# huangzh13/StyleGAN.pytorch

Measured on AMD Instinct MI355X. Metric: img/s full G+D train step, 1024x1024 depth-9 bf16, higher is better.
Workload: dtype bf16; 1 GPU; ffhq1024: StyleGAN 1024x1024, progressive depth index 8, logistic+R1, alpha 0.5, batch 4/GPU, global batch 4; global_batch=4, parallelism=dp1

## Files before the change

### include/sgx.h

```cpp
#ifndef SGX_H
#define SGX_H
#include <stddef.h>
#include <stdint.h>
#ifdef __cplusplus
extern "C" {
#endif

enum { SGX_F32 = 0, SGX_BF16 = 1 };
enum { SGX_ACT_NONE = 0, SGX_ACT_LRELU = 1, SGX_ACT_RELU = 2 };
enum { SGX_EINVAL = -1, SGX_EUNSUPPORTED = -2, SGX_EWORKSPACE = -3 };

int sgx_version(void);
const char* sgx_last_error(void);
int sgx_clear_error(void);
int sgx_stream_wait_stream(void* waiter, void* signaler);
int sgx_selftest_tr16(void* out256, void* stream);

int sgx_prof_start(int mode, int only_of);
int sgx_prof_count(void);
int sgx_prof_get(int i, char* name, int name_cap, float* ms, double* flops, double* bytes, char* desc, int desc_cap);

int sgx_conv3x3(const void* x, const void* w, const float* bias, void* y, int B, int H, int W, int Cin, int Cout,
                int act, const void* mask, int dtype, void* stream);
int sgx_conv4x4s2_down(const void* x, const void* w, const float* bias, void* y, int B, int H, int W, int Cin,
                       int Cout, int act, int dtype, void* stream);
int sgx_conv4x4s2_up(const void* x, const void* w, void* y, int B, int H, int W, int Cin, int Cout, int dtype,
                     void* stream);
int sgx_conv_variant(int geo, const void* x, const void* w, const float* bias, void* y, int B, int H, int W, int Cin, int Cout,
                     int act, int dtype, int variant, void* stream);
size_t sgx_conv_splitk_ws_bytes(int geo, int B, int H, int W, int Cin, int Cout, int dtype);
int sgx_conv_splitk(int geo, const void* x, const void* w, const float* bias, void* y, const void* mask, int B, int H, int W, int Cin, int Cout,
                    int act, int dtype, void* ws, size_t ws_bytes, void* stream);

int sgx_conv_config(int geo, int B, int H, int W, int Cin, int Cout, int dtype, int* cfg5);
enum { SGX_PACK_S = 0, SGX_PACK_D = 1, SGX_PACK_U = 2, SGX_PACK_UF = 3 };
int sgx_pack_weight(const float* w, void* fwd, void* adj, int O, int I, int Ipad, int mode, float scale, int dtype,
                    void* stream);
#define SGX_PACK_ROW 10
int sgx_pack_weight_blocks(int O, int Ipad);
int sgx_pack_weight_multi(const void* table, int n, int total_blocks, int dtype, void* stream);
size_t sgx_wgrad_ws_bytes(int taps, int B, int H, int W, int Ck, int Cn);
int sgx_wgrad3x3_param(const void* x, const void* dy, float* dW, float* db, void* ws, size_t ws_bytes, int B, int H, int W,
                       int Cx, int Cdy, int adjoint, float scale, int O, int I, int accumulate, int dtype, void* stream);
int sgx_wgrad4x4s2_param(const void* fine, const void* coarse, float* dW, float* db, void* ws, size_t ws_bytes, int B, int H,
                         int W, int Cfine, int Ccoarse, int mode, float scale, int O, int I, int accumulate, int dtype,
                         void* stream);

int sgx_bias_act(const void* x, const float* bias, float bscale, void* y, size_t npix, int C, int act, int dtype,
                 void* stream);
int sgx_lrelu_bwd(const void* dy, const void* y, void* dx, size_t n, float slope, float scale, const float* scale_dev, int dtype,
                  void* stream);
int sgx_lrelu_bwd_bits(const void* dy, const void* bits, void* dx, size_t n, float slope, float scale, const float* scale_dev, int dtype,
                       void* stream);
int sgx_conv4x4s2_down_fade_ok(int B, int H, int W, int Cin, int Cout, int dtype);
int sgx_conv4x4s2_down_fade(const void* x, const void* w, const float* bias, const void* resid, float alpha, float beta, const float* ab_dev,
                            void* y, void* bits, int B, int H, int W, int Cin, int Cout, int dtype, void* stream);
int sgx_conv4x4s2_down_fade_rgb(const void* x, const void* w, const float* bias, const float* pimg, const float* wr, float ws, const float* rb,
                                float bs1, float bs2, float alpha, float beta, const float* ab_dev, void* y, void* bits, int B, int H, int W,
                                int Cin, int Cout, int dtype, void* stream);
size_t sgx_fade_rgb_bwd_ws_bytes(size_t npix, int C);
int sgx_fade_rgb_bwd(const void* g, const void* bits, const float* pimg, const float* wr, float ws, float bs, float alpha, float beta,
                     const float* ab_dev, void* gy, float* dwr, float* drb, int acc, float* gpimg, void* wsbuf, size_t ws_bytes, size_t npix, int C,
                     int dtype, void* stream);
int sgx_fade_rgb_bwd_finish(const void* wsbuf, size_t ws_bytes, size_t npix, int C, float ws, float bs, float beta, const float* ab_dev,
                            float* dwr, float* drb, int acc, void* stream);
int sgx_fade_rgb_bwd2(const void* ggy, const float* ggp, const void* bits, const float* wr, float ws, float alpha, float beta, const float* ab_dev,
                      void* out, size_t npix, int C, int dtype, void* stream);
int sgx_axpby(const void* a, const void* b, void* out, float alpha, float beta, size_t n, int dtype, void* stream);
int sgx_axpby_dev(const void* a, const void* b, void* out, const float* alpha_dev, const float* beta_dev, size_t n, int dtype,
                  void* stream);
int sgx_blur3x3(const void* x, void* y, int B, int H, int W, int C, int dtype, void* stream);
int sgx_blur3x3_act(const void* x, const void* z, void* y, int B, int H, int W, int C, int mode, int dtype, void* stream);
int sgx_blur3x3_bits(const void* x, const void* bits, void* y, int B, int H, int W, int C, int mode, int dtype, void* stream);
int sgx_blur_kxk(const void* x, void* y, const float* taps_host, int K, int pad, int B, int IH, int IW, int OH, int OW, int C,
                 int dtype, void* stream);
int sgx_images_u8_to_nhwc(const void* src, void* dst, const int* flip, int B, int H, int W, int src_chw, int dtype, void* stream);
int sgx_pool2(const void* x, void* y, int B, int H, int W, int C, float scale, int dtype, void* stream);
int sgx_up2(const void* x, void* y, int B, int H, int W, int C, float scale, int dtype, void* stream);
int sgx_up2_add(const void* x, const void* a, void* y, int B, int H, int W, int C, float scale, int dtype, void* stream);
size_t sgx_colsum_ws_bytes(size_t npix, int C);
int sgx_colsum(const void* x, float* out, float scale, void* ws, size_t ws_bytes, size_t npix, int C, int dtype,
               void* stream);

int sgx_rgb_in(const float* img, const float* w, int sj, int sc, float wscale, const float* bias, void* y, size_t npix,
               int C, int dtype, void* stream);
int sgx_rgb_out(const void* x, const float* w, int sj, int sc, float wscale, const float* bias, float* img, size_t npix,
                int C, int dtype, void* stream);
int sgx_rgb_in_add(const float* img, const float* w, int sj, int sc, float wscale, const void* add, void* y, size_t npix, int C, int dtype,
                   void* stream);
size_t sgx_rgb_wgrad_ws_bytes(size_t npix, int C);
int sgx_downsample_fade_rgb(const float* x, float* out, int B, int H, int W, float alpha, float beta, const float* ab_dev, void* stream);
size_t sgx_diffaug_ws_bytes(int B, int H, int W);
int sgx_diffaug(const float* x, float* y, const float* u, int B, int H, int W, int policy_bits, int adjoint, int with_bias, void* ws,
                size_t ws_bytes, void* stream);
int sgx_rgb_out_fade(const void* x, const float* w, int sj, int sc, float wscale, const float* bias, const float* low, float alpha,
                     float beta, const float* ab_dev, float* img, int B, int H, int W, int C, int dtype, void* stream);
int sgx_rgb_wgrad(const float* img, const void* f, float* dw, int sj, int sc, float wscale, void* ws, size_t ws_bytes,
                  size_t npix, int C, int dtype, void* stream);

enum { SGX_EPI_ACT = 1, SGX_EPI_NORM = 2 };
size_t sgx_gepi_ws_bytes(int B, int HW, int C);
int sgx_gepi_fwd(const void* x, const float* bias, const float* noise, const float* nw, const float* style, void* y,
                 float* mean, float* rstd, void* ws, size_t ws_bytes, const double* pre_part, int pre_npart, int B, int HW,
                 int C, int flags, int dtype, void* stream);
int sgx_blur3x3_stats_nparts(int B, int H, int W, int C, int dtype);
int sgx_conv3x3_stats_nparts(int B, int H, int W, int Cin, int Cout, int dtype);
int sgx_conv3x3_signbits_ok(int B, int H, int W, int Cin, int Cout, int dtype);
int sgx_conv3x3_signbits(const void* x, const void* w, const float* bias, void* y, void* bits, int B, int H, int W, int Cin, int Cout,
                         int act, const void* mask, int dtype, void* stream);
int sgx_conv4x4s2_up_blur_ok(int B, int H, int W, int Cin, int Cout, int dtype);
int sgx_conv4x4s2_up_blur(const void* x, const void* w, void* y, const void* mask, int B, int H, int W, int Cin, int Cout,
                          int dtype, void* stream);
int sgx_pack_upblur(const float* w, void* wc, int O, int I, int mode, int adjoint, float scale, void* stream);
int sgx_conv_upblur_ok(int B, int H, int W, int Cin, int Cout, int dtype);
int sgx_conv_upblur(const void* x, const void* wc, void* y, const void* maskbits, int B, int H, int W, int Cin, int Cout, int dtype, void* stream);
int sgx_conv4x4s2_up_blur_bits(const void* x, const void* w, void* y, const void* bits, int B, int H, int W, int Cin, int Cout,
                               int dtype, void* stream);
int sgx_conv3x3_stats(const void* x, const void* w, void* y, const float* ebias, const float* noise, const float* nw, double* part,
                      size_t part_bytes, int B, int H, int W, int Cin, int Cout, int dtype, void* stream);

int sgx_rgbconv_ok(int B, int H, int W, int C, int dtype);
int sgx_rgbconv_pack(const float* w0, float s0, const float* wr, float sr, const float* br, float bscale, void* wf, void* wd, int C,
                     void* stream);
int sgx_rgbconv_fwd(const float* img, const void* wf, const float* b0, void* y, void* bits, int B, int H, int W, int C, int epi, int ones,
                    int dtype, void* stream);
int sgx_rgbconv_tune(int fwd_variant, int nit, int dbg);
int sgx_rgbconv_dgrad(const void* gz, const void* wd, float* gi, int B, int H, int W, int C, int dtype, void* stream);
size_t sgx_rgbconv_wgrad_ws_bytes(int B, int H, int W, int C);
int sgx_rgbconv_wgrad(const float* img, const void* gz, int ones, const float* w0, float s0, const float* wr, float sr, const float* br,
                      float bscale, float* dw0, float* db0, float* dwr, float* dbr, int acc, void* ws, size_t ws_bytes, int B, int H, int W,
                      int C, int dtype, void* stream);
int sgx_blur3x3_stats(const void* x, void* y, const float* bias, const float* noise, const float* nw, double* part,
                      size_t part_bytes, int B, int H, int W, int C, int act, int dtype, void* stream);
int sgx_gepi_bwd(const void* dy, const void* x, const float* bias, const float* noise, const float* nw,
                 const float* style, const float* mean, const float* rstd, void* dx, float* dstyle, float* dnw,
                 float* dbias, void* ws, size_t ws_bytes, int B, int HW, int C, int flags, int dtype, void* stream);

int sgx_pixelnorm_fwd(const float* x, float* y, int B, int C, void* stream);
int sgx_pixelnorm_bwd(const float* dy, const float* x, float* dx, int B, int C, void* stream);
int sgx_mbstd_fwd(const void* x, void* y, int B, int HW, int C, int Cpad, int dtype, void* stream);
int sgx_mbstd_bwd(const void* dy, const void* x, void* dx, int B, int HW, int C, int Cpad, int dtype, void* stream);
int sgx_mbstd_bwd2(const void* ggx, const void* dy, const void* x, void* ddy, void* gx, int B, int HW, int C, int Cpad,
                   int dtype, void* stream);
size_t sgx_sumsq_ws_bytes(void);
int sgx_sumsq_f32(const float* x, size_t n, void* ws, size_t ws_bytes, float* out, void* stream);
int sgx_scale_dev_f32(const float* x, const float* s, float alpha, float* out, size_t n, void* stream);
int sgx_logistic_loss(const float* fake, int n_fake, const float* real, int n_real, float scale, int generator, float* loss,
                      float* g_fake, float* g_real, void* stream);
size_t sgx_gemm_ws_bytes(int M, int N, int K);
int sgx_gemm_f32(const float* A, const float* Bm, float* C, int M, int N, int K, int ta, int tb, float alpha,
                 void* ws, size_t ws_bytes, void* stream);
int sgx_linear_fwd(const float* x, const float* w, const float* bias, float* y, int B, int N, int K, float w_mul, float b_mul,
                   int act, void* stream);
int sgx_linear_bwd_data(const float* gy, const float* y_act, const float* w, float* gx, int B, int N, int K, float w_mul,
                        void* stream);
int sgx_linear_bwd_param(const float* gy, const float* y_act, const float* x, float* dw, float* db, int B, int N, int K, float w_mul,
                         float b_mul, void* stream);
#define SGX_STYLE_ROW 8
int sgx_style_fwd(const float* lm, const void* table, float* y, int G, int B, int D, int total_tiles, void* stream);
int sgx_style_bwd_data(const float* gy, const void* table, float* glm, int G, int B, int D, int max_n, void* stream);
int sgx_style_bwd_param(const float* gy, const float* lm, const void* table, float* dw, float* db, int G, int B, int D,
                        int total_tiles, void* stream);

int sgx_gepi_stats(const void* x, const float* bias, const float* noise, const float* nw, float* mean, float* rstd, void* ws, size_t ws_bytes,
                   const double* pre_part, int pre_npart, int B, int HW, int C, int flags, int dtype, void* stream);
int sgx_rgb_out_epi(const void* y, const float* ebias, const float* noise, const float* nw, const float* style, const float* mean,
                    const float* rstd, const float* w, int sj, int sc, float wscale, const float* rbias, const float* low, float alpha, float beta,
                    const float* ab_dev, float* img, int B, int H, int W, int C, int dtype, void* stream);
size_t sgx_rgb_wgrad_epi_ws_bytes(int B, int HW, int C);
int sgx_rgb_wgrad_epi(const void* y, const float* g, const float* ebias, const float* noise, const float* nw, const float* style, const float* mean,
                      const float* rstd, float* dw, float* db, int sj, int sc, float scale, float bscale, void* ws, size_t ws_bytes, int B, int HW,
                      int C, int dtype, void* stream);

int sgx_adam_multi(float* const* params, const float* const* grads, float* const* exp_avg, float* const* exp_avg_sq,
                   const int64_t* sizes, int n, float beta1, float beta2, float eps, const float* step_sizes,
                   const float* bc2_sqrts, const float* grad_scale, void* stream);
int sgx_ema_multi(float* const* tgt, const float* const* src, const int64_t* sizes, int n, float beta, void* stream);
int sgx_gradnorm_clip_coef(const float* const* grads, const int64_t* sizes, int n, float max_norm, double* partial,
                           float* out, void* stream);

#ifdef __cplusplus
}
#endif
#endif
```

### stylegan/pytorch_amd/Blocks.py

```python
import os

import torch
import torch.nn as nn

from . import functional as F
from .CustomLayers import (BlurLayer, EqualizedConv2d, EqualizedLinear, LayerEpilogue, StddevLayer, View, act_code, apply_act)
from .native import ACT_LRELU, ACT_NONE


FUSE_EPI_STATS = int(os.environ.get("SGX_FUSE_EPI_STATS", "2"))
FUSE_EPI_STATS_MIN = int(os.environ.get("SGX_FUSE_EPI_STATS_MIN", str(1 << 27)))


FUSE_BLUR_BWD = os.environ.get("SGX_FUSE_BLUR_BWD", "1") != "0"


def _lat(d, k):
    return d[k] if isinstance(d, (tuple, list)) else d[:, k]


class InputBlock(nn.Module):

    def __init__(self, nf, dlatent_size, const_input_layer, gain, use_wscale, use_noise, use_pixel_norm,
                 use_instance_norm, use_styles, activation_layer):
# ... 19 lines not shown
            x = self.const.permute(0, 2, 3, 1).to(dtype).expand(b, -1, -1, -1).contiguous()
            bias = self.bias
        else:
            x = self.dense(_lat(dlatents_in_range, 0)).view(b, self.nf, 4, 4).permute(0, 2, 3, 1).to(dtype).contiguous()
            bias = None
        x = self.epi1.forward_nhwc(x, _lat(dlatents_in_range, 0), conv_bias=bias)
        x = self.conv.forward_nhwc(x, skip_bias=True)
        return self.epi2.forward_nhwc(x, _lat(dlatents_in_range, 1), conv_bias=self.conv.scaled_bias())

    def forward(self, dlatents_in_range):
        return F.nchw_view(self.forward_nhwc(dlatents_in_range))


class GSynthesisBlock(nn.Module):

    def __init__(self, in_channels, out_channels, blur_filter, dlatent_size, gain, use_wscale, use_noise,
                 use_pixel_norm, use_instance_norm, use_styles, activation_layer):
        super().__init__()
        blur = BlurLayer(blur_filter) if blur_filter else None
        self.conv0_up = EqualizedConv2d(in_channels, out_channels, kernel_size=3, gain=gain, use_wscale=use_wscale,
                                        intermediate=blur, upscale=True)
        self.epi1 = LayerEpilogue(out_channels, dlatent_size, use_wscale, use_noise, use_pixel_norm,
                                  use_instance_norm, use_styles, activation_layer)
        self.conv1 = EqualizedConv2d(out_channels, out_channels, kernel_size=3, gain=gain, use_wscale=use_wscale)
        self.epi2 = LayerEpilogue(out_channels, dlatent_size, use_wscale, use_noise, use_pixel_norm,
                                  use_instance_norm, use_styles, activation_layer)

    def forward_nhwc(self, x, dlatents_in_range, defer_epi2=False):
        up = self.conv0_up
        if (FUSE_EPI_STATS & 1) and self.epi1._fusable and up.intermediate is not None and up.intermediate._is_121:
            b, h, w, _ = x.shape
            nin = self.epi1.noise_inputs((b, 2 * h, 2 * w, up.weight.shape[0]), x.device)
            x, part = up.forward_nhwc(x, skip_bias=True, epi_stats=(up.scaled_bias(),) + nin)
            x = self.epi1.forward_nhwc(x, _lat(dlatents_in_range, 0), conv_bias=up.scaled_bias(), noise_in=nin, pre_stats=part)
        else:
            x = up.forward_nhwc(x, skip_bias=True)
            x = self.epi1.forward_nhwc(x, _lat(dlatents_in_range, 0), conv_bias=up.scaled_bias())
        defer_epi2 = defer_epi2 and self.epi2._fusable
        if (FUSE_EPI_STATS & 2) and self.epi2._fusable and x.numel() >= FUSE_EPI_STATS_MIN:
            nin = self.epi2.noise_inputs(x.shape, x.device)
            x, part = self.conv1.forward_nhwc(x, skip_bias=True, epi_stats=(self.conv1.scaled_bias(),) + nin)
            if defer_epi2:
                return x, (self.conv1.scaled_bias(), nin[0], nin[1], self.epi2._style(_lat(dlatents_in_range, 1)), part)
            return self.epi2.forward_nhwc(x, _lat(dlatents_in_range, 1), conv_bias=self.conv1.scaled_bias(), noise_in=nin, pre_stats=part)
        if defer_epi2:
            nin = self.epi2.noise_inputs(x.shape, x.device)
            x = self.conv1.forward_nhwc(x, skip_bias=True)
            return x, (self.conv1.scaled_bias(), nin[0], nin[1], self.epi2._style(_lat(dlatents_in_range, 1)), None)
        x = self.conv1.forward_nhwc(x, skip_bias=True)
        return self.epi2.forward_nhwc(x, _lat(dlatents_in_range, 1), conv_bias=self.conv1.scaled_bias())

    def forward(self, x, dlatents_in_range):
        return F.nchw_view(self.forward_nhwc(F.nhwc(x), dlatents_in_range))


class DiscriminatorTop(nn.Module):

    def __init__(self, mbstd_group_size, mbstd_num_features, in_channels, intermediate_channels, gain, use_wscale,
                 activation_layer, resolution=4, in_channels2=None, output_features=1, last_gain=1):
        super().__init__()
        if mbstd_group_size > 1:
            self.stddev_layer = StddevLayer(mbstd_group_size, mbstd_num_features)
        else:
            self.stddev_layer = None
        if in_channels2 is None:
            in_channels2 = in_channels
        nfeat = mbstd_num_features if mbstd_group_size > 1 else 0
        self.conv = EqualizedConv2d(in_channels + nfeat, in_channels2, kernel_size=3, gain=gain, use_wscale=use_wscale)
        self.act0 = activation_layer
        self.view = View(-1)
        self.dense0 = EqualizedLinear(in_channels2 * resolution * resolution, intermediate_channels, gain=gain,
                                      use_wscale=use_wscale)
        self.act1 = activation_layer
        self.dense1 = EqualizedLinear(intermediate_channels, output_features, gain=last_gain, use_wscale=use_wscale)
        self.resolution = resolution
        self._act = act_code(activation_layer)

    def forward_nhwc(self, x):
        fused = ACT_LRELU if self._act == ACT_LRELU else ACT_NONE
        post = ACT_NONE if fused else self._act
        if self.stddev_layer is not None:
            x = self.stddev_layer.forward_nhwc(x)
        x = apply_act(self.conv.forward_nhwc(x, act=fused), post)
        b = x.shape[0]
        flat = x.permute(0, 3, 1, 2).reshape(b, -1).float()
        y = apply_act(self.dense0(flat, act=fused), post)
        return self.dense1(y)

    def forward(self, x):
        return self.forward_nhwc(F.nhwc(x))


class DiscriminatorBlock(nn.Module):

    def __init__(self, in_channels, out_channels, gain, use_wscale, activation_layer, blur_kernel):
        super().__init__()
        self.conv0 = EqualizedConv2d(in_channels, in_channels, kernel_size=3, gain=gain, use_wscale=use_wscale)
        self.act0 = activation_layer
        self.blur = BlurLayer(kernel=blur_kernel)
        self.conv1_down = EqualizedConv2d(in_channels, out_channels, kernel_size=3, gain=gain, use_wscale=use_wscale,
                                          downscale=True)
        self.act1 = activation_layer
        self._act = act_code(activation_layer)

    def fused_from_rgb_ok(self, img_shape, from_rgb, dtype):
        c0 = self.conv0
        return (FUSE_BLUR_BWD and self.blur._is_121 and self._act == ACT_LRELU and len(img_shape) == 4 and img_shape[3] == 3
                and from_rgb.kernel_size == 1 and tuple(from_rgb.weight.shape[1:]) == (3, 1, 1) and c0.b_mul == 1 and from_rgb.b_mul == 1
                and from_rgb.weight.shape[0] == c0.weight.shape[1] == c0.weight.shape[0]
                and F.rgbconv_ok(img_shape[0], img_shape[1], img_shape[2], c0.weight.shape[0], dtype))

    def forward_from_image(self, img, from_rgb, defer_out=False, fade=None):
        c0 = self.conv0
        xb, zbits = F.rgbconv_blur(img, c0.weight, c0.scaled_bias(), from_rgb.weight, from_rgb.scaled_bias(), c0.w_mul, from_rgb.w_mul)
        if fade is not None and F.conv_down_fade_ok(xb, self.conv1_down.weight.shape[0]):
            return self.conv1_down.forward_nhwc(xb, act=ACT_LRELU, x_pre=None, x_pre_bits=zbits, fade=fade), True
        y = self.conv1_down.forward_nhwc(xb, act=ACT_LRELU, defer_act=defer_out and self._act == ACT_LRELU, x_pre=None, x_pre_bits=zbits)
        return (y, False) if fade is not None else y

    def forward_nhwc(self, x, x_masked=False, defer_out=False, fade=None):
        x_masked = x_masked and self._act == ACT_LRELU
        defer_out = defer_out and self._act == ACT_LRELU
        if self.blur._is_121 and self._act == ACT_LRELU and FUSE_BLUR_BWD:
            z, zbits = self.conv0.forward_nhwc(x, act=ACT_NONE, x_masked=x_masked, sign_bits=True)
            x = F.act_blur_pass(z)
            if fade is not None and F.conv_down_fade_ok(x, self.conv1_down.weight.shape[0]):
                return self.conv1_down.forward_nhwc(x, act=ACT_LRELU, x_pre=z, x_pre_bits=zbits, fade=fade), True
            y = self.conv1_down.forward_nhwc(x, act=ACT_LRELU, defer_act=defer_out, x_pre=z, x_pre_bits=zbits)
            return (y, False) if fade is not None else y
        z = self.conv0.forward_nhwc(x, act=ACT_NONE, x_masked=x_masked)
        if self.blur._is_121 and self._act == ACT_LRELU:
            x = F.call(F.ActBlurFn, z)
        else:
            x = self.blur.forward_nhwc(apply_act(z, self._act))
        if self._act == ACT_LRELU:
            y = self.conv1_down.forward_nhwc(x, act=ACT_LRELU, defer_act=defer_out)
        else:
            y = apply_act(self.conv1_down.forward_nhwc(x, act=ACT_NONE), self._act)
        return (y, False) if fade is not None else y

    def forward(self, x):
        return F.nchw_view(self.forward_nhwc(F.nhwc(x)))
```

### stylegan/pytorch_amd/CustomLayers.py

```python
import math

import numpy as np
import torch
import torch.nn as nn

from . import functional as F
from .native import ACT_LRELU, ACT_NONE, ACT_RELU, EPI_ACT, EPI_NORM

MBSTD_CPAD = 32


def act_code(activation_layer):
    if isinstance(activation_layer, nn.LeakyReLU) and abs(activation_layer.negative_slope - 0.2) < 1e-12:
        return ACT_LRELU
    if activation_layer is torch.relu or isinstance(activation_layer, nn.ReLU):
        return ACT_RELU
    raise NotImplementedError(f"activation {activation_layer!r}: the reference offers 'lrelu' (0.2) and 'relu'")


def apply_act(x, act):
    return F.call(F.BiasActFn, x, None, 1.0, act) if act else x


class PixelNormLayer(nn.Module):
# ... 40 lines not shown
        k = torch.tensor(kernel, dtype=torch.float32)
        k = k[:, None] * k[None, :]
        k = k[None, None]
        if normalize:
            k = k / k.sum()
        if flip:
            k = k.flip(2, 3)
        self.register_buffer('kernel', k)
        self.stride = stride
        self._is_121 = (list(kernel) == [1, 2, 1]) and normalize and stride == 1
        self._is_box2 = (len(kernel) == 2 and stride == 2 and abs(float(k.sum()) - 1.0) < 1e-6
                         and float((k - k.mean()).abs().max()) < 1e-7)
        self._taps = None

    def _host_taps(self):
        ver = self.kernel._version
        if self._taps is None or self._taps[0] != ver:
            k = self.kernel.detach().float().cpu()
            self._taps = (ver, int(k.shape[2]), tuple(float(v) for v in k.reshape(-1)))
        return self._taps[1], self._taps[2]

    def forward_nhwc(self, x):
        if self._is_121:
            return F.call(F.BlurFn, x)
        if self._is_box2:
            return F.call(F.Pool2Fn, x, 0.25)
        if self.stride != 1:
            raise NotImplementedError("BlurLayer: stride 2 is built for the 2x2 box of Downscale2d only")
        K, taps = self._host_taps()
        if K > 7:
            raise NotImplementedError("BlurLayer: filters longer than 7 taps are not built")
        pad = int((K - 1) / 2)
        return F.call(F.BlurGenFn, x, taps, K, pad, x.shape[1] + 2 * pad - K + 1, x.shape[2] + 2 * pad - K + 1)

    def forward(self, x):
        return F.nchw_view(self.forward_nhwc(F.nhwc(x)))


class Downscale2d(nn.Module):

    def __init__(self, factor=2, gain=1):
        super().__init__()
        assert isinstance(factor, int) and factor >= 1
        self.factor = factor
        self.gain = gain
        if factor == 2:
            f = [np.sqrt(gain) / factor] * factor
            self.blur = BlurLayer(kernel=f, normalize=False, stride=factor)
        else:
            self.blur = None

    def forward_nhwc(self, x):
        assert self.factor == 2, "the kernel implements the factor-2 case the networks use"
        return F.call(F.Pool2Fn, x, 0.25 * float(self.gain))

    def forward(self, x):
        assert x.dim() == 4
        return F.nchw_view(self.forward_nhwc(F.nhwc(x)))


class EqualizedLinear(nn.Module):

    first_order_only = False

    def __init__(self, input_size, output_size, gain=2 ** 0.5, use_wscale=False, lrmul=1, bias=True):
        super().__init__()
        he_std = gain * input_size ** (-0.5)
        if use_wscale:
            init_std = 1.0 / lrmul
            self.w_mul = he_std * lrmul
        else:
            init_std = he_std / lrmul
            self.w_mul = lrmul
        self.weight = nn.Parameter(torch.randn(output_size, input_size) * init_std)
        if bias:
            self.bias = nn.Parameter(torch.zeros(output_size))
            self.b_mul = lrmul
        else:
            self.bias = None
            self.b_mul = 1

    def forward(self, x, act=ACT_NONE, weight=None):
        w = self.weight if weight is None else weight
        if self.first_order_only and x.dim() == 2:
            return F.linear_fused(x.float(), w, self.bias, self.w_mul, self.b_mul, act)
        return F.linear(x.float(), w, self.bias, self.w_mul, self.b_mul, act)


class EqualizedConv2d(nn.Module):

    def __init__(self, input_channels, output_channels, kernel_size, stride=1, gain=2 ** 0.5, use_wscale=False,
                 lrmul=1, bias=True, intermediate=None, upscale=False, downscale=False):
        super().__init__()
        self.upscale = Upscale2d() if upscale else None
        self.downscale = Downscale2d() if downscale else None
        he_std = gain * (input_channels * kernel_size ** 2) ** (-0.5)
        self.kernel_size = kernel_size
        if use_wscale:
            init_std = 1.0 / lrmul
            self.w_mul = he_std * lrmul
        else:
            init_std = he_std / lrmul
            self.w_mul = lrmul
        self.weight = nn.Parameter(torch.randn(output_channels, input_channels, kernel_size, kernel_size) * init_std)
        if bias:
            self.bias = nn.Parameter(torch.zeros(output_channels))
            self.b_mul = lrmul
        else:
            self.bias = None
            self.b_mul = 1
        self.intermediate = intermediate
        assert stride == 1

    def scaled_bias(self):
        if self.bias is None:
            return None
        return self.bias * self.b_mul if self.b_mul != 1 else self.bias

    def forward_nhwc(self, x, act=ACT_NONE, skip_bias=False, out_dtype=None, defer_act=False, x_masked=False, out_scale=1.0,
                     epi_stats=None, x_pre=None, sign_bits=False, x_pre_bits=None, fade=None):
        bias = None if skip_bias else self.scaled_bias()
        cin, cout = self.weight.shape[1], self.weight.shape[0]
        if self.kernel_size == 1:
            assert self.upscale is None and self.downscale is None and self.intermediate is None
            if cin == 3 and x.shape[3] == 3:
                if out_scale != 1.0:
                    y = F.call(F.RgbInFn, x.float(), self.weight, None if bias is None else bias * float(out_scale),
                               self.w_mul * float(out_scale), out_dtype or torch.float32)
                else:
                    y = F.call(F.RgbInFn, x.float(), self.weight, bias, self.w_mul, out_dtype or torch.float32)
            elif cin % 3 == 0 and cin > 3 and x.shape[3] == cin and cout != 3:
                y = None
                for k in range(0, cin, 3):
                    part = F.call(F.RgbInFn, x[..., k:k + 3].float().contiguous(), self.weight[:, k:k + 3].contiguous(),
                                  bias if k == 0 else None, self.w_mul, out_dtype or torch.float32)
                    y = part if y is None else F.call(F.AxpbyFn, y, part, 1.0, 1.0)
            elif cout == 3:
                y = F.call(F.RgbOutFn, x, self.weight, bias, self.w_mul)
            else:
                raise NotImplementedError("1x1 EqualizedConv2d is built for the to_rgb / from_rgb layers (3 channels on one side)")
            return F.call(F.BiasActFn, y, None, 1.0, act) if act else y
        assert self.kernel_size == 3
        if epi_stats is not None:
            assert skip_bias and act == ACT_NONE and self.downscale is None
            ebias, noise, nw = epi_stats
            if self.upscale is not None:
                fused = min(x.shape[1], x.shape[2]) * 2 >= 128
                y = F.conv(x, self.weight, None, "U" if fused else "UF", self.w_mul)
                assert self.intermediate is not None and self.intermediate._is_121
                return F.call(F.BlurStatsFn, y, ebias, noise, nw)
            assert self.intermediate is None
            if F.conv_stats_nparts(x, self.weight.shape[0]) > 0:
                return F.conv(x, self.weight, None, "S", self.w_mul, ipad=x.shape[3], stats=(ebias, noise, nw))
            return F.conv(x, self.weight, None, "S", self.w_mul, ipad=x.shape[3]), None
        if self.upscale is not None:
            fused = min(x.shape[1], x.shape[2]) * 2 >= 128
            mode = "U" if fused else "UF"
            if (self.intermediate is not None and self.intermediate._is_121
                    and F.conv_blur_ok(x, self.weight.shape[0], mode, False)):
                y = F.call(F.ConvBlurFn, x, self.weight, mode, float(self.w_mul), int(self.weight.shape[1]), False, None)
            else:
                y = F.conv(x, self.weight, None, mode, self.w_mul)
                if self.intermediate is not None:
                    y = self.intermediate.forward_nhwc(y)
            if bias is not None or act:
                y = F.call(F.BiasActFn, y, bias, 1.0, act)
# ... 172 lines not shown
```

### stylegan/pytorch_amd/GAN.py

```python
import contextlib
import copy
import datetime
import os
import random
import time
import timeit
from collections import OrderedDict

import numpy as np
import torch
import torch.nn as nn

from . import Losses
from . import functional as F
from .Blocks import DiscriminatorBlock, DiscriminatorTop, GSynthesisBlock, InputBlock
from .CustomLayers import EqualizedConv2d, EqualizedLinear, PixelNormLayer, Truncation, act_code, apply_act
from .data import get_data_loader
from . import native
from .native import ACT_LRELU
from .optim import FusedAdam, clip_and_step, ema_update


class DeferredLoss:

# ... 5 lines not shown
            with torch.cuda.stream(stream) if stream is not None else contextlib.nullcontext():
                t = dev_scalar.detach().reshape(1).float()
                view, slot = native.RING.take(4)
                self._host = view.view(torch.float32)
                self._host.copy_(t, non_blocking=True)
                self._event = native.RING.mark(slot, owner=self)
        else:
            self._host, self._event = dev_scalar.detach().reshape(1).float().clone(), None

    def item(self):
        if self._value is None:
            if self._event is not None:
                self._event.synchronize()
            self._value = float(self._host[0]) * self._scale
        return self._value

    __float__ = item

    def __format__(self, spec): return format(self.item(), spec)
    def __repr__(self): return repr(self.item())
    def __add__(self, o): return self.item() + float(o)
    __radd__ = __add__
    def __sub__(self, o): return self.item() - float(o)
    def __rsub__(self, o): return float(o) - self.item()
    def __mul__(self, o): return self.item() * float(o)
    __rmul__ = __mul__
    def __truediv__(self, o): return self.item() / float(o)
    def __lt__(self, o): return self.item() < float(o)
    def __gt__(self, o): return self.item() > float(o)
    def __eq__(self, o): return self.item() == float(o)
    def __abs__(self): return abs(self.item())
    def __neg__(self): return -self.item()
    def __hash__(self): return hash(self.item())


FUSE_RGB_FADE = os.environ.get("SGX_FUSE_RGB_FADE", "1") != "0"


def _nonlinearity(name):
    return {'relu': (nn.ReLU(), np.sqrt(2)), 'lrelu': (nn.LeakyReLU(negative_slope=0.2), np.sqrt(2))}[name]


def _conv_weights(module):
    ws = module.__dict__.get("_sgx_conv_weights")
    if ws is None:
        ws = [m.weight for m in module.modules() if isinstance(m, EqualizedConv2d)]
        module.__dict__["_sgx_conv_weights"] = ws
    return ws


def update_average(model_tgt, model_src, beta):
    ema_update(model_tgt, model_src, beta)


class GMapping(nn.Module):

    def __init__(self, latent_size=512, dlatent_size=512, dlatent_broadcast=None, mapping_layers=8, mapping_fmaps=512,
                 mapping_lrmul=0.01, mapping_nonlinearity='lrelu', use_wscale=True, normalize_latents=True, **kwargs):
        super().__init__()
        self.latent_size = latent_size
        self.mapping_fmaps = mapping_fmaps
        self.dlatent_size = dlatent_size
        self.dlatent_broadcast = dlatent_broadcast
        act, gain = _nonlinearity(mapping_nonlinearity)
        self._act = act_code(act)
        layers = []
        if normalize_latents:
            layers.append(('pixel_norm', PixelNormLayer()))
        layers.append(('dense0', EqualizedLinear(self.latent_size, self.mapping_fmaps, gain=gain, lrmul=mapping_lrmul,
                                                 use_wscale=use_wscale)))
        layers.append(('dense0_act', act))
        for layer_idx in range(1, mapping_layers):
            fmaps_in = self.mapping_fmaps
            fmaps_out = self.dlatent_size if layer_idx == mapping_layers - 1 else self.mapping_fmaps
            layers.append(('dense{:d}'.format(layer_idx),
                           EqualizedLinear(fmaps_in, fmaps_out, gain=gain, lrmul=mapping_lrmul, use_wscale=use_wscale)))
            layers.append(('dense{:d}_act'.format(layer_idx), act))
        self.map = nn.Sequential(OrderedDict(layers))
        self.mapping_layers = mapping_layers
        for m in self.map.modules():
            if isinstance(m, EqualizedLinear):
                m.first_order_only = True

    def forward(self, x):
        x = x.float()
        if hasattr(self.map, 'pixel_norm'):
            x = self.map.pixel_norm(x)
        for i in range(self.mapping_layers):
            dense = getattr(self.map, 'dense{:d}'.format(i))
            if self._act == ACT_LRELU:
                x = dense(x, act=ACT_LRELU)
            else:
                x = apply_act(dense(x), self._act)
        if self.dlatent_broadcast is not None:
            x = x.unsqueeze(1).expand(-1, self.dlatent_broadcast, -1)
        return x


class GSynthesis(nn.Module):

    def __init__(self, dlatent_size=512, num_channels=3, resolution=1024, fmap_base=8192, fmap_decay=1.0, fmap_max=512,
                 use_styles=True, const_input_layer=True, use_noise=True, nonlinearity='lrelu', use_wscale=True,
                 use_pixel_norm=False, use_instance_norm=True, blur_filter=None, structure='linear', act_dtype=torch.float32,
                 **kwargs):
        super().__init__()

        def nf(stage):
            return min(int(fmap_base / (2.0 ** (stage * fmap_decay))), fmap_max)

        self.structure = structure
        resolution_log2 = int(np.log2(resolution))
        assert resolution == 2 ** resolution_log2 and resolution >= 4
        self.depth = resolution_log2 - 1
        self.num_layers = resolution_log2 * 2 - 2
        self.num_styles = self.num_layers if use_styles else 1
        self.act_dtype = act_dtype
        act, gain = _nonlinearity(nonlinearity)

        self.init_block = InputBlock(nf(1), dlatent_size, const_input_layer, gain, use_wscale, use_noise, use_pixel_norm,
                                     use_instance_norm, use_styles, act)
        rgb_converters = [EqualizedConv2d(nf(1), num_channels, 1, gain=1, use_wscale=use_wscale)]
        blocks = []
        for res in range(3, resolution_log2 + 1):
            last_channels = nf(res - 2)
            channels = nf(res - 1)
            blocks.append(GSynthesisBlock(last_channels, channels, blur_filter, dlatent_size, gain, use_wscale, use_noise,
                                          use_pixel_norm, use_instance_norm, use_styles, act))
            rgb_converters.append(EqualizedConv2d(channels, num_channels, 1, gain=1, use_wscale=use_wscale))
        self.blocks = nn.ModuleList(blocks)
        self.to_rgb = nn.ModuleList(rgb_converters)
        self.temporaryUpsampler = lambda x: F.nchw_view(F.call(F.Up2Fn, F.nhwc(x), 1.0))

    def forward(self, dlatents_in, depth=0, alpha=0., labels_in=None):
        assert depth < self.depth, "Requested output depth cannot be produced"
        F.prepack(_conv_weights(self))
        dl = self._styles(dlatents_in.float(), depth)
        dt = self.act_dtype
        nblocks = len(self.blocks) if self.structure == 'fixed' else depth
        prev_arena = F.NOISE_ARENA
        if any(m.noise is None for m in self._noise_layers()):
            b = dlatents_in.shape[0]
            F.NOISE_ARENA = F.NoiseArena(b * sum(2 * (4 << k) ** 2 for k in range(nblocks + 1)), dlatents_in.device)
        try:
            return self._forward(dl, dt, depth, alpha)
        finally:
            F.NOISE_ARENA = prev_arena

    def _styles(self, dlatents, depth):
        nblocks = len(self.blocks) if self.structure == 'fixed' else depth
        epis = [self.init_block.epi1, self.init_block.epi2]
        for blk in self.blocks[:nblocks]:
            epis += [blk.epi1, blk.epi2]
        B = dlatents.shape[0]
        ok = (getattr(self.init_block, "const_input_layer", False) and B <= 32 and dlatents.shape[2] % 64 == 0
              and all(getattr(e, "_fusable", False) and e.style_mod is not None for e in epis))
        if not ok:
            return F.call(F.SplitLayersFn, dlatents)
        lins = [e.style_mod.lin for e in epis]
        meta = tuple((i, float(l.w_mul), float(l.b_mul)) for i, l in enumerate(lins))
        lm = dlatents.transpose(0, 1).contiguous()
        styles = F.call(F.GroupedStyleFn, lm, meta, *[l.weight for l in lins], *[l.bias for l in lins])
        return [F.PreStyle(s) for s in styles] + [None] * (dlatents.shape[1] - len(styles))

    def _noise_layers(self):
        ls = self.__dict__.get("_sgx_noise_layers")
        if ls is None:
            from .CustomLayers import NoiseLayer
            ls = self.__dict__["_sgx_noise_layers"] = [m for m in self.modules() if isinstance(m, NoiseLayer)]
        return ls

    def _forward(self, dl, dt, depth, alpha):
        if self.structure == 'fixed':
            x = self.init_block.forward_nhwc(dl[0:2], dt)
            rgb, last = self.to_rgb[-1], (self.blocks[-1] if len(self.blocks) else None)
            fuse_last = (F.FUSE_EPI_RGB and last is not None and last.epi2._fusable and rgb.weight.shape[0] == 3
                         and F.epi_rgb_out_ok(rgb.weight.shape[1], self.act_dtype))
            for i, block in enumerate(self.blocks):
                if fuse_last and block is last:
                    y2, (ebias, noise, nw, style, part) = block.forward_nhwc(x, dl[2 * (i + 1):2 * (i + 2)], defer_epi2=True)
                    return F.nchw_view(F.call(F.EpiRgbOutFn, y2, ebias, noise, nw, style, rgb.weight, rgb.scaled_bias(), float(rgb.w_mul), None, 1.0, part))
                x = block.forward_nhwc(x, dl[2 * (i + 1):2 * (i + 2)])
            images = rgb.forward_nhwc(x)
        elif self.structure == 'linear':
            x = self.init_block.forward_nhwc(dl[0:2], dt)
            if depth > 0:
                for i, block in enumerate(self.blocks[:depth - 1]):
                    x = block.forward_nhwc(x, dl[2 * (i + 1):2 * (i + 2)])
                prev = self.to_rgb[depth - 1]
                if F.RGB_FORK and prev.weight.shape[0] == 3 and prev.weight.shape[1] == x.shape[3]:
                    x, low = F.call(F.RgbOutForkFn, x, prev.weight, prev.scaled_bias(), prev.w_mul)
                else:
                    low = prev.forward_nhwc(x)
                rgb = self.to_rgb[depth]
                last = self.blocks[depth - 1]
                if (F.FUSE_EPI_RGB and FUSE_RGB_FADE and last.epi2._fusable and rgb.weight.shape[0] == 3 and low.dtype == torch.float32
                        and F.epi_rgb_out_ok(rgb.weight.shape[1], x.dtype)):
                    y2, (ebias, noise, nw, style, part) = last.forward_nhwc(x, dl[2 * depth:2 * (depth + 1)], defer_epi2=True)
                    return F.nchw_view(F.call(F.EpiRgbOutFn, y2, ebias, noise, nw, style, rgb.weight, rgb.scaled_bias(), float(rgb.w_mul), low,
                                              alpha if isinstance(alpha, torch.Tensor) else float(alpha), part))
                xs = last.forward_nhwc(x, dl[2 * depth:2 * (depth + 1)])
                if FUSE_RGB_FADE and rgb.weight.shape[0] == 3 and low.dtype == torch.float32:
                    images = F.call(F.RgbOutFadeFn, xs, rgb.weight, rgb.scaled_bias(), float(rgb.w_mul), low, alpha)
                else:
                    images = F.fade(rgb.forward_nhwc(xs), F.call(F.Up2Fn, low, 1.0), alpha)
            else:
                images = self.to_rgb[0].forward_nhwc(x)
        else:
            raise KeyError("Unknown structure: ", self.structure)
        return F.nchw_view(images)


class Generator(nn.Module):

    def __init__(self, resolution, latent_size=512, dlatent_size=512, conditional=False, n_classes=0, truncation_psi=0.7,
                 truncation_cutoff=8, dlatent_avg_beta=0.995, style_mixing_prob=0.9, **kwargs):
        super().__init__()
        if conditional:
            assert n_classes > 0, "Conditional generation requires n_class > 0"
            self.class_embedding = nn.Embedding(n_classes, latent_size)
            latent_size *= 2
        self.conditional = conditional
        self.style_mixing_prob = style_mixing_prob
        self.num_layers = (int(np.log2(resolution)) - 1) * 2
        self.g_mapping = GMapping(latent_size, dlatent_size, dlatent_broadcast=self.num_layers, **kwargs)
        self.g_synthesis = GSynthesis(resolution=resolution, **kwargs)
        if truncation_psi > 0:
            self.truncation = Truncation(avg_latent=torch.zeros(dlatent_size), max_layer=truncation_cutoff,
                                         threshold=truncation_psi, beta=dlatent_avg_beta)
        else:
            self.truncation = None

    _mixing_override = None
    _avg_latent_hook = None

    def draw_mixing_host(self, shape, depth):
        latents2 = torch.randn(shape)
        cur_layers = 2 * (depth + 1)
        cutoff = random.randint(1, cur_layers) if random.random() < self.style_mixing_prob else cur_layers
        return latents2, cutoff

    def draw_mixing(self, shape, depth, device):
        latents2, cutoff = self.draw_mixing_host(shape, depth)
        if device.type == "cuda":
            latents2 = native.upload(latents2.contiguous(), device)[0]
        return latents2, cutoff

    def forward(self, latents_in, depth, alpha, labels_in=None):
        if self.conditional:
            assert labels_in is not None, "Conditional discriminatin requires labels"
            latents_in = torch.cat([latents_in, self.class_embedding(labels_in)], 1)
        mixing = self.training and self.style_mixing_prob is not None and self.style_mixing_prob > 0
        if mixing:
            latents2, mixing_cutoff = self._mixing_override or self.draw_mixing(latents_in.shape, depth, latents_in.device)
            both = self.g_mapping(torch.cat([latents_in, latents2.to(latents_in.dtype)], 0))
            dlatents_in, dlatents2 = both[:latents_in.shape[0]], both[latents_in.shape[0]:]
        else:
            dlatents_in = self.g_mapping(latents_in)
        if self.training:
            if self.truncation is not None:
                self.truncation.update(dlatents_in[0, 0].detach())
                if self._avg_latent_hook is not None:
                    self._avg_latent_hook(self.truncation.avg_latent)
            if mixing:
                layer_idx = torch.arange(self.num_layers, device=latents_in.device).view(1, -1, 1)
                dlatents_in = torch.where(layer_idx < mixing_cutoff, dlatents_in, dlatents2)
            if self.truncation is not None:
                dlatents_in = self.truncation(dlatents_in)
        return self.g_synthesis(dlatents_in, depth, alpha)


class Discriminator(nn.Module):

    def __init__(self, resolution, num_channels=3, conditional=False, n_classes=0, fmap_base=8192, fmap_decay=1.0,
                 fmap_max=512, nonlinearity='lrelu', use_wscale=True, mbstd_group_size=4, mbstd_num_features=1,
                 blur_filter=None, structure='linear', act_dtype=torch.float32, diffaug_policy="", **kwargs):
        super().__init__()
        self.diffaug_policy = diffaug_policy or ""
        self._diffaug_bits = F.diffaug_policy_bits(self.diffaug_policy)
        if conditional:
            assert n_classes > 0, "Conditional Discriminator requires n_class > 0"
            num_channels *= 2
        embeddings = []

        def nf(stage):
            return min(int(fmap_base / (2.0 ** (stage * fmap_decay))), fmap_max)

        self.conditional = conditional
        self.mbstd_num_features = mbstd_num_features
        self.mbstd_group_size = mbstd_group_size
        self.structure = structure
        self.act_dtype = act_dtype
        resolution_log2 = int(np.log2(resolution))
        assert resolution == 2 ** resolution_log2 and resolution >= 4
        self.depth = resolution_log2 - 1
        act, gain = _nonlinearity(nonlinearity)

        blocks, from_rgb = [], []
        for res in range(resolution_log2, 2, -1):
            blocks.append(DiscriminatorBlock(nf(res - 1), nf(res - 2), gain=gain, use_wscale=use_wscale,
                                             activation_layer=act, blur_kernel=blur_filter))
            from_rgb.append(EqualizedConv2d(num_channels, nf(res - 1), kernel_size=1, gain=gain, use_wscale=use_wscale))
            if conditional:
                r = 2 ** res
                embeddings.append(nn.Embedding(n_classes, (num_channels // 2) * r * r))
        if conditional:
            embeddings.append(nn.Embedding(n_classes, (num_channels // 2) * 4 * 4))
            self.embeddings = nn.ModuleList(embeddings)
        self.blocks = nn.ModuleList(blocks)
        self.final_block = DiscriminatorTop(self.mbstd_group_size, self.mbstd_num_features, in_channels=nf(2),
                                            intermediate_channels=nf(2), gain=gain, use_wscale=use_wscale,
                                            activation_layer=act)
        from_rgb.append(EqualizedConv2d(num_channels, nf(2), kernel_size=1, gain=gain, use_wscale=use_wscale))
        self.from_rgb = nn.ModuleList(from_rgb)
        self.temporaryDownsampler = lambda x: F.nchw_view(F.call(F.Pool2Fn, F.nhwc(x), 0.25))

    diffaug_override = None

    def _diffaug(self, img):
        u = self.diffaug_override
        if u is None:
            u = torch.rand(img.shape[0], 7, device=img.device)
        return F.call(F.DiffAugFn, img, u, self._diffaug_bits)

    def prepack(self, depth=None, img_shape=None):
        F.prepack(_conv_weights(self))
        if depth is not None and img_shape is not None and self.structure == 'linear' and depth > 0 and not self.conditional:
            top, top_rgb = self.blocks[self.depth - depth - 1], self.from_rgb[self.depth - depth - 1]
            if top.fused_from_rgb_ok(img_shape, top_rgb, self.act_dtype):
                F.rgb_packs(top.conv0.weight, top.conv0.w_mul, top_rgb.weight, top_rgb.w_mul, top_rgb.scaled_bias())

    def forward(self, images_in, depth, alpha=1., labels_in=None):
        assert depth < self.depth, "Requested output depth cannot be produced"
        img = F.nhwc(images_in, torch.float32)
        if self._diffaug_bits and self.training:
            img = self._diffaug(img)
        self.prepack(depth, img.shape)
# ... 742 lines not shown
```

### stylegan/pytorch_amd/csrc/pointwise.hip

```cpp
#include "common.h"

static inline unsigned grid_for(size_t nvec, int block = 256) {
    size_t g = (nvec + block - 1) / block;
    static const size_t cap = [] { const char* e = getenv("SGX_GRID_CAP"); const long v = e ? atol(e) : 8192; return (size_t)(v > 0 ? v : 0x7fffffffL); }();
    if (g > cap) g = cap;
    if (g < 1) g = 1;
    return (unsigned)g;
}
static inline unsigned grid_all(size_t nvec, int block = 256) {
    size_t g = (nvec + block - 1) / block;
    static const size_t cap = [] { const char* e = getenv("SGX_GRID_ALL_CAP"); const long v = e ? atol(e) : 0; return (size_t)(v > 0 ? v : 0x7fffffffL); }();
    if (g > cap) g = cap;
    if (g < 1) g = 1;
    return (unsigned)g;
}

template <typename T>
__global__ void bias_act_kernel(const T* __restrict__ x, const float* __restrict__ bias, float bscale, T* __restrict__ y,
                                size_t nvec, int C, int act) {
    constexpr int VE = VecTraits<T>::VE;
    const int cv = C / VE;
    for (size_t i = (size_t)blockIdx.x * blockDim.x + threadIdx.x; i < nvec; i += (size_t)gridDim.x * blockDim.x) {
        float v[VE];
        VecTraits<T>::load(x + i * VE, v);
// ... 947 lines not shown
            const int e = q * 4 + j;
            v[j] = ae[j] + scale * src[((e / 3) >> 1) * 3 + e % 3];
        }
        *reinterpret_cast<float4*>(y + row * OW * 3 + q * 4) = make_float4(v[0], v[1], v[2], v[3]);
    }
}
template <typename T>
__global__ void up2_add_kernel(const T* __restrict__ x, const T* __restrict__ a, T* __restrict__ y, int B, int H, int W, int C, float scale) {
    const int OH = 2 * H, OW = 2 * W;
    const size_t n = (size_t)B * OH * OW * C;
    for (size_t i = (size_t)blockIdx.x * blockDim.x + threadIdx.x; i < n; i += (size_t)gridDim.x * blockDim.x) {
        const int c = (int)(i % C);
        size_t p = i / C;
        const int ow = (int)(p % OW); p /= OW;
        const int oh = (int)(p % OH);
        const int b = (int)(p / OH);
        y[i] = from_f<T>(to_f(a[i]) + scale * to_f(x[(((size_t)b * H + (oh >> 1)) * W + (ow >> 1)) * C + c]));
    }
}
extern "C" int sgx_up2_add(const void* x, const void* a, void* y, int B, int H, int W, int C, float scale, int dtype, void* stream) {
    hipStream_t st = (hipStream_t)stream;
    SGX_REQUIRE(x && a && y && B > 0 && H > 0 && W > 0 && C > 0, SGX_EINVAL, "up2_add: bad arguments");
    SGX_REQUIRE(dtype == SGX_F32 || dtype == SGX_BF16, SGX_EINVAL, "up2_add: bad dtype");
    const double es = dtype == SGX_F32 ? 4.0 : 2.0;
    SGX_NOTE(0.0, 9.0 * es * B * H * W * C, "up2+add B%d %dx%d C%d", B, H, W, C);
    const size_t nout = (size_t)B * H * W * 4 * C;
    if (dtype == SGX_F32 && C == 3 && (2 * W * 3) % 4 == 0)
        hipLaunchKernelGGL(up2_add_rgb_kernel, dim3(grid_all(nout / 4)), dim3(256), 0, st, (const float*)x, (const float*)a, (float*)y, B, H, W, scale);
    else if (dtype == SGX_F32)
        hipLaunchKernelGGL(up2_add_kernel<float>, dim3(grid_for(nout)), dim3(256), 0, st, (const float*)x, (const float*)a, (float*)y, B, H, W, C, scale);
    else
        hipLaunchKernelGGL(up2_add_kernel<bf16_t>, dim3(grid_for(nout)), dim3(256), 0, st, (const bf16_t*)x, (const bf16_t*)a, (bf16_t*)y, B, H, W, C, scale);
    SGX_LAUNCH_CHECK("up2_add");
    return 0;
}
extern "C" int sgx_up2(const void* x, void* y, int B, int H, int W, int C, float scale, int dtype, void* stream) {
    hipStream_t st = (hipStream_t)stream;
    SGX_NOTE(0.0, 5.0 * (dtype == SGX_F32 ? 4.0 : 2.0) * B * H * W * C, "up2 B%d %dx%d C%d", B, H, W, C);
    const size_t nout = (size_t)B * H * W * 4 * C;
    if (dtype == SGX_F32) {
        if (C % 4 == 0) hipLaunchKernelGGL((up2_kernel<float, true>), dim3(grid_all(nout / 4)), dim3(256), 0, st, (const float*)x, (float*)y, B, H, W, C, scale);
        else if (C == 3 && W % 4 == 0 && (reinterpret_cast<uintptr_t>(x) & 15) == 0 && (reinterpret_cast<uintptr_t>(y) & 15) == 0)
            hipLaunchKernelGGL(up2_rgb4_kernel, dim3(grid_all((size_t)B * H * (W / 4))), dim3(256), 0, st, (const float*)x, (float*)y, B, H, W, scale);
        else if (C == 3 && (2 * W * 3) % 4 == 0) hipLaunchKernelGGL(up2_rgb_kernel, dim3(grid_all(nout / 4)), dim3(256), 0, st, (const float*)x, (float*)y, B, H, W, scale);
        else hipLaunchKernelGGL((up2_kernel<float, false>), dim3(grid_for(nout)), dim3(256), 0, st, (const float*)x, (float*)y, B, H, W, C, scale);
    } else {
        if (C % 8 == 0) hipLaunchKernelGGL((up2_kernel<bf16_t, true>), dim3(grid_all(nout / 8)), dim3(256), 0, st, (const bf16_t*)x, (bf16_t*)y, B, H, W, C, scale);
        else hipLaunchKernelGGL((up2_kernel<bf16_t, false>), dim3(grid_for(nout)), dim3(256), 0, st, (const bf16_t*)x, (bf16_t*)y, B, H, W, C, scale);
    }
    SGX_LAUNCH_CHECK("up2");
    return 0;
}

#define COLSUM_BLOCKS 1024
template <typename T>
__global__ void colsum_stage1(const T* __restrict__ x, double* __restrict__ ws, size_t npix, int C) {
    extern __shared__ double sh[];
    const int tpr = C < 256 ? C : 256;
    const int rows = 256 / tpr;
    const int tc = threadIdx.x % tpr, tr = threadIdx.x / tpr;
    const size_t per = (npix + gridDim.x - 1) / gridDim.x;
    const size_t p0 = (size_t)blockIdx.x * per, p1 = (p0 + per < npix) ? p0 + per : npix;
    for (int cb = 0; cb < C; cb += tpr) {
        const int c = cb + tc;
        double acc = 0.0;
        if (tr < rows && c < C) {
            float part = 0.f; int cnt = 0;
            for (size_t p = p0 + tr; p < p1; p += rows) {
                part += to_f(x[p * C + c]);
                if (++cnt == 64) { acc += (double)part; part = 0.f; cnt = 0; }
            }
            acc += (double)part;
        }
        sh[threadIdx.x] = acc;
        __syncthreads();
        if (tr == 0 && c < C) {
            double s = 0.0;
            for (int r = 0; r < rows; ++r) s += sh[r * tpr + tc];
            ws[(size_t)blockIdx.x * C + c] = s;
        }
        __syncthreads();
    }
}
__global__ __launch_bounds__(256) void colsum_stage2(const double* __restrict__ ws, float* __restrict__ out, int nblk, int C, float scale) {
    __shared__ double sh[64][5];
    const int cl = threadIdx.x & 3, pl = threadIdx.x >> 2;
    const int c = blockIdx.x * 4 + cl;
    double s = 0.0;
    if (c < C)
        for (int b = pl; b < nblk; b += 64) s += ws[(size_t)b * C + c];
    sh[pl][cl] = s;
    __syncthreads();
    if (pl == 0 && c < C) {
        double t = 0.0;
        for (int k = 0; k < 64; ++k) t += sh[k][cl];
        out[c] = (float)(t * (double)scale);
    }
}
template <typename T, int NJ>
__global__ __launch_bounds__(256) void colsum_vec_stage1(const T* __restrict__ x, const float* __restrict__ img, double* __restrict__ ws,
                                                         size_t npix, int C) {
    constexpr int VE = VecTraits<T>::VE;
    extern __shared__ float shf[];
    const int cv = C / VE, rows = 256 / cv;
    const int tc = threadIdx.x % cv, tr = threadIdx.x / cv;
    const size_t per = (npix + gridDim.x - 1) / gridDim.x;
    const size_t p0 = (size_t)blockIdx.x * per, p1 = (p0 + per < npix) ? p0 + per : npix;
    float part[NJ * VE];
#pragma unroll
    for (int k = 0; k < NJ * VE; ++k) part[k] = 0.f;
    auto accum = [&](const float (&v)[VE], size_t p) {
        if (NJ == 1) {
#pragma unroll
            for (int k = 0; k < VE; ++k) part[k] += v[k];
        } else {
            const float r = img[p * 3], g = img[p * 3 + 1], b = img[p * 3 + 2];
#pragma unroll
            for (int k = 0; k < VE; ++k) { part[k] += v[k] * r; part[VE + k] += v[k] * g; part[2 * VE + k] += v[k] * b; }
        }
    };
    size_t p = p0 + tr;
    for (; p + 3 * (size_t)rows < p1; p += 4 * (size_t)rows) {
        float v0[VE], v1[VE], v2[VE], v3[VE];
        VecTraits<T>::load(x + (p * cv + tc) * VE, v0);
        VecTraits<T>::load(x + ((p + rows) * cv + tc) * VE, v1);
        VecTraits<T>::load(x + ((p + 2 * (size_t)rows) * cv + tc) * VE, v2);
        VecTraits<T>::load(x + ((p + 3 * (size_t)rows) * cv + tc) * VE, v3);
        accum(v0, p); accum(v1, p + rows); accum(v2, p + 2 * (size_t)rows); accum(v3, p + 3 * (size_t)rows);
    }
    for (; p < p1; p += rows) {
        float v[VE];
        VecTraits<T>::load(x + (p * cv + tc) * VE, v);
        accum(v, p);
    }
#pragma unroll
    for (int k = 0; k < NJ * VE; ++k) shf[threadIdx.x * NJ * VE + k] = part[k];
    __syncthreads();
    for (int o = threadIdx.x; o < cv * NJ * VE; o += 256) {
        const int c = o / (NJ * VE), k = o % (NJ * VE);
        double s = 0.0;
        for (int r = 0; r < rows; ++r) s += (double)shf[(r * cv + c) * NJ * VE + k];
        ws[((size_t)blockIdx.x * NJ + k / VE) * C + c * VE + (k % VE)] = s;
    }
}
static bool colsum_vec_ok(int C, int ve) { const int cv = C / ve; return C % ve == 0 && cv >= 1 && cv <= 256 && (cv & (cv - 1)) == 0; }

extern "C" size_t sgx_colsum_ws_bytes(size_t npix, int C) { (void)npix; return (size_t)COLSUM_BLOCKS * C * sizeof(double); }
extern "C" int sgx_colsum(const void* x, float* out, float scale, void* ws, size_t ws_bytes, size_t npix, int C, int dtype, void* stream) {
    hipStream_t st = (hipStream_t)stream;
    SGX_REQUIRE(ws_bytes >= sgx_colsum_ws_bytes(npix, C), SGX_EWORKSPACE, "colsum: workspace");
    SGX_REQUIRE(C >= 1, SGX_EINVAL, "colsum: C=%d", C);
    SGX_NOTE(0.0, (dtype == SGX_F32 ? 4.0 : 2.0) * npix * C, "colsum %zux%d", npix, C);
    int nblk = (int)((npix + 63) / 64);
    if (nblk > COLSUM_BLOCKS) nblk = COLSUM_BLOCKS;
    if (nblk < 1) nblk = 1;
    if (dtype == SGX_F32 && colsum_vec_ok(C, 4))
        hipLaunchKernelGGL((colsum_vec_stage1<float, 1>), dim3(nblk), dim3(256), 256 * 4 * sizeof(float), st, (const float*)x, (const float*)nullptr, (double*)ws, npix, C);
    else if (dtype == SGX_BF16 && colsum_vec_ok(C, 8))
        hipLaunchKernelGGL((colsum_vec_stage1<bf16_t, 1>), dim3(nblk), dim3(256), 256 * 8 * sizeof(float), st, (const bf16_t*)x, (const float*)nullptr, (double*)ws, npix, C);
    else if (dtype == SGX_F32) hipLaunchKernelGGL(colsum_stage1<float>, dim3(nblk), dim3(256), 256 * sizeof(double), st, (const float*)x, (double*)ws, npix, C);
    else hipLaunchKernelGGL(colsum_stage1<bf16_t>, dim3(nblk), dim3(256), 256 * sizeof(double), st, (const bf16_t*)x, (double*)ws, npix, C);
    SGX_LAUNCH_CHECK("colsum_stage1");
    hipLaunchKernelGGL(colsum_stage2, dim3((C + 3) / 4), dim3(256), 0, st, (const double*)ws, out, nblk, C, scale);
    SGX_LAUNCH_CHECK("colsum_stage2");
    return 0;
}

template <typename T>
__global__ void rgb_in_kernel(const float* __restrict__ img, const float* __restrict__ w, int sj, int sc, float wscale,
                              const float* __restrict__ bias, T* __restrict__ y, size_t npix, int C, const T* __restrict__ add) {
    constexpr int VE = VecTraits<T>::VE;
    const int cv = C / VE;
    const size_t nvec = npix * cv;
    const size_t i0 = (size_t)blockIdx.x * blockDim.x + threadIdx.x;
    const int c0 = (int)(i0 % cv) * VE;
    float wr[VE], wg[VE], wb[VE], bb[VE];
#pragma unroll
    for (int j = 0; j < VE; ++j) {
        wr[j] = wscale * w[(c0 + j) * sc]; wg[j] = wscale * w[sj + (c0 + j) * sc]; wb[j] = wscale * w[2 * sj + (c0 + j) * sc];
        bb[j] = bias ? bias[c0 + j] : 0.f;
    }
    for (size_t i = i0; i < nvec; i += (size_t)gridDim.x * blockDim.x) {
        const size_t p = i / cv;
        const float r = img[p * 3], g = img[p * 3 + 1], b = img[p * 3 + 2];
        float v[VE];
#pragma unroll
        for (int j = 0; j < VE; ++j) v[j] = bb[j] + (r * wr[j] + g * wg[j] + b * wb[j]);
        if (add) {
            float av[VE];
            VecTraits<T>::load(add + i * VE, av);
#pragma unroll
            for (int j = 0; j < VE; ++j) v[j] += av[j];
        }
        VecTraits<T>::store(y + i * VE, v);
    }
}
template <typename T>
__global__ __launch_bounds__(256) void rgb_in1_kernel(const float* __restrict__ img, const float* __restrict__ w, int sj, int sc, float wscale,
                                                      const float* __restrict__ bias, T* __restrict__ y, unsigned nvec, int C, const T* __restrict__ add) {
    constexpr int VE = VecTraits<T>::VE, U = 4;
    extern __shared__ float tw[];
    for (int c = threadIdx.x; c < C; c += 256) {
        tw[c] = wscale * w[c * sc]; tw[C + c] = wscale * w[sj + c * sc]; tw[2 * C + c] = wscale * w[2 * sj + c * sc];
        tw[3 * C + c] = bias ? bias[c] : 0.f;
    }
    const unsigned i0 = blockIdx.x * (256u * U) + threadIdx.x, cv = (unsigned)(C / VE);
    float r[U], g[U], b[U];
    uint4 araw[U];
#pragma unroll
    for (int u = 0; u < U; ++u) {
        const unsigned i = i0 + u * 256u;
        r[u] = g[u] = b[u] = 0.f; araw[u] = make_uint4(0u, 0u, 0u, 0u);
        if (i < nvec) {
            const size_t p = i / cv;
            r[u] = img[p * 3]; g[u] = img[p * 3 + 1]; b[u] = img[p * 3 + 2];
            if (add) araw[u] = *reinterpret_cast<const uint4*>(add + (size_t)i * VE);
        }
    }
    __syncthreads();
#pragma unroll
    for (int u = 0; u < U; ++u) {
        const unsigned i = i0 + u * 256u;
        if (i >= nvec) continue;
        const int c0 = (int)(i % cv) * VE;
        float v[VE];
#pragma unroll
        for (int j = 0; j < VE; ++j) v[j] = tw[3 * C + c0 + j] + (r[u] * tw[c0 + j] + g[u] * tw[C + c0 + j] + b[u] * tw[2 * C + c0 + j]);
        if (add) {
            const unsigned w4[4] = {araw[u].x, araw[u].y, araw[u].z, araw[u].w};
            if constexpr (sizeof(T) == 2) {
#pragma unroll
                for (int k = 0; k < 4; ++k) { v[(2 * k) % VE] += __uint_as_float(w4[k] << 16); v[(2 * k + 1) % VE] += __uint_as_float(w4[k] & 0xffff0000u); }
            } else {
#pragma unroll
                for (int k = 0; k < 4; ++k) v[k % VE] += __uint_as_float(w4[k]);
            }
        }
        VecTraits<T>::store(y + (size_t)i * VE, v);
    }
}
template <typename T>
static bool rgb_in1_launch(const float* img, const float* w, int sj, int sc, float wscale, const float* bias, T* y, size_t npix, int C, const T* add, hipStream_t st) {
    static const int on = [] { const char* e = getenv("SGX_RGB_IN1"); return e ? atoi(e) : 1; }();
    const size_t nvec = npix * (C / VecTraits<T>::VE);
    if (!on || nvec < 65536 || nvec >= 0x7fffffffull || C > 2048) return false;
    hipLaunchKernelGGL(rgb_in1_kernel<T>, dim3((unsigned)((nvec + 1023) / 1024)), dim3(256), (size_t)4 * C * sizeof(float), st, img, w, sj, sc, wscale, bias, y,
// ... 461 lines not shown
```

### stylegan/pytorch_amd/csrc/small.hip

```cpp
#include "common.h"

__global__ void pixelnorm_fwd_kernel(const float* __restrict__ x, float* __restrict__ y, int B, int C) {
    const int row = blockIdx.x * (blockDim.x / 64) + threadIdx.x / 64, lane = threadIdx.x & 63;
    if (row >= B) return;
    float ss = 0.f;
    for (int c = lane; c < C; c += 64) { const float v = x[(size_t)row * C + c]; ss += v * v; }
    ss = wave_sum(ss);
    const float r = rsqrtf(ss / C + 1e-8f);
    for (int c = lane; c < C; c += 64) y[(size_t)row * C + c] = x[(size_t)row * C + c] * r;
}
__global__ void pixelnorm_bwd_kernel(const float* __restrict__ dy, const float* __restrict__ x, float* __restrict__ dx, int B, int C) {
    const int row = blockIdx.x * (blockDim.x / 64) + threadIdx.x / 64, lane = threadIdx.x & 63;
    if (row >= B) return;
    float ss = 0.f, dot = 0.f;
    for (int c = lane; c < C; c += 64) {
        const float v = x[(size_t)row * C + c];
        ss += v * v; dot += v * dy[(size_t)row * C + c];
    }
    ss = wave_sum(ss); dot = wave_sum(dot);
    const float r = rsqrtf(ss / C + 1e-8f);
    const float k = r * r * r * dot / C;
    for (int c = lane; c < C; c += 64) dx[(size_t)row * C + c] = dy[(size_t)row * C + c] * r - x[(size_t)row * C + c] * k;
}
extern "C" int sgx_pixelnorm_fwd(const float* x, float* y, int B, int C, void* stream) {
// ... 111 lines not shown
    for (int i0 = threadIdx.x; i0 < n; i0 += MBSTD_U * blockDim.x) {
        float v[MBSTD_U][4], gg[MBSTD_U][4];
#pragma unroll
        for (int u = 0; u < MBSTD_U; ++u) {
            const int i = i0 + u * blockDim.x, ii = i < n ? i : n - 1;
#pragma unroll
            for (int g = 0; g < 4; ++g) {
                const size_t o = (size_t)((g < G ? g : 0) * M + m) * n + ii;
                v[u][g] = to_f(x[o]); gg[u][g] = to_f(ggx[o]);
            }
        }
#pragma unroll
        for (int u = 0; u < MBSTD_U; ++u)
            if (i0 + u * (int)blockDim.x < n) {
                float mu = 0.f;
                MBSTD_FOR_G(g) mu += v[u][g];
                mu /= G;
                float var = 0.f, dot = 0.f;
                MBSTD_FOR_G(g) {
                    const float d = v[u][g] - mu;
                    var += d * d;
                    dot += d * gg[u][g];
                }
                a_dd += (double)(dot / sqrtf(var / G + 1e-8f));
            }
    }
    const float k = (float)(block_sum_d(a_gy, sh) / n) / G;
    const float dstat = (float)(block_sum_d(a_dd, sh) / n) / G;
    for (int i = blockIdx.y * blockDim.x + threadIdx.x; i < n; i += gridDim.y * blockDim.x) {
        float v[4], gg[4], mu = 0.f;
#pragma unroll
        for (int g = 0; g < 4; ++g) {
            const size_t o = (size_t)((g < G ? g : 0) * M + m) * n + i;
            v[g] = to_f(x[o]); gg[g] = to_f(ggx[o]);
        }
        MBSTD_FOR_G(g) mu += v[g];
        mu /= G;
        float var = 0.f, dot = 0.f;
        MBSTD_FOR_G(g) { const float d = v[g] - mu; var += d * d; dot += d * gg[g]; }
        const float s = sqrtf(var / G + 1e-8f);
        float u[4], um = 0.f;
        MBSTD_FOR_G(g) { u[g] = gg[g] / s - dot * (v[g] - mu) / (G * s * s * s); um += u[g]; }
        um /= G;
        MBSTD_FOR_G(g) gx[(size_t)(g * M + m) * n + i] = from_f<T>(k * (u[g] - um));
    }
    mbstd_padded_copy(ggx, ddy, dstat, G, M, m, HW, C, Cpad);
}

#ifndef MBSTD_NB
#define MBSTD_NB 8
#endif
static int mbstd_check(int B, int C, int Cpad) {
    SGX_REQUIRE(B > 0 && (B < 4 || B % 4 == 0), SGX_EINVAL, "mbstd: batch %d not divisible by group size", B);
    SGX_REQUIRE(Cpad > C, SGX_EINVAL, "mbstd: Cpad must exceed C");
    return 0;
}
extern "C" int sgx_mbstd_fwd(const void* x, void* y, int B, int HW, int C, int Cpad, int dtype, void* stream) {
    int rc = mbstd_check(B, C, Cpad); if (rc) return rc;
    const int M = B / (B < 4 ? B : 4);
    if (dtype == SGX_F32) hipLaunchKernelGGL(mbstd_fwd_kernel<float>, dim3(M, MBSTD_NB), dim3(1024), 0, (hipStream_t)stream, (const float*)x, (float*)y, B, HW, C, Cpad);
    else hipLaunchKernelGGL(mbstd_fwd_kernel<bf16_t>, dim3(M, MBSTD_NB), dim3(1024), 0, (hipStream_t)stream, (const bf16_t*)x, (bf16_t*)y, B, HW, C, Cpad);
    SGX_LAUNCH_CHECK("mbstd_fwd");
    return 0;
}
extern "C" int sgx_mbstd_bwd(const void* dy, const void* x, void* dx, int B, int HW, int C, int Cpad, int dtype, void* stream) {
    int rc = mbstd_check(B, C, Cpad); if (rc) return rc;
    const int M = B / (B < 4 ? B : 4);
    if (dtype == SGX_F32) hipLaunchKernelGGL(mbstd_bwd_kernel<float>, dim3(M, MBSTD_NB), dim3(1024), 0, (hipStream_t)stream, (const float*)dy, (const float*)x, (float*)dx, B, HW, C, Cpad);
    else hipLaunchKernelGGL(mbstd_bwd_kernel<bf16_t>, dim3(M, MBSTD_NB), dim3(1024), 0, (hipStream_t)stream, (const bf16_t*)dy, (const bf16_t*)x, (bf16_t*)dx, B, HW, C, Cpad);
    SGX_LAUNCH_CHECK("mbstd_bwd");
    return 0;
}
extern "C" int sgx_mbstd_bwd2(const void* ggx, const void* dy, const void* x, void* ddy, void* gx, int B, int HW, int C, int Cpad,
                              int dtype, void* stream) {
    int rc = mbstd_check(B, C, Cpad); if (rc) return rc;
    const int M = B / (B < 4 ? B : 4);
    if (dtype == SGX_F32) hipLaunchKernelGGL(mbstd_bwd2_kernel<float>, dim3(M, MBSTD_NB), dim3(1024), 0, (hipStream_t)stream, (const float*)ggx, (const float*)dy, (const float*)x, (float*)ddy, (float*)gx, B, HW, C, Cpad);
    else hipLaunchKernelGGL(mbstd_bwd2_kernel<bf16_t>, dim3(M, MBSTD_NB), dim3(1024), 0, (hipStream_t)stream, (const bf16_t*)ggx, (const bf16_t*)dy, (const bf16_t*)x, (bf16_t*)ddy, (bf16_t*)gx, B, HW, C, Cpad);
    SGX_LAUNCH_CHECK("mbstd_bwd2");
    return 0;
}

struct GemmFuse { const float* amask; const float* bias; float bscale; int act; float* colsum; float cscale; };
template <bool VA, bool VB, bool MASK, bool TAIL>
__device__ __forceinline__ void gemm_step_load(const float* __restrict__ A, const float* __restrict__ am, const float* __restrict__ Bm,
                                               size_t arow, size_t sa_k, size_t bcol, size_t sb_k, int kk, int ke, float (&a4)[4],
                                               float (&b4)[4]) {
    if (VA && !TAIL) {
        const float4 t = *reinterpret_cast<const float4*>(A + arow + kk);
        a4[0] = t.x; a4[1] = t.y; a4[2] = t.z; a4[3] = t.w;
        if (MASK) {
            const float4 m = *reinterpret_cast<const float4*>(am + arow + kk);
            a4[0] *= lrelu_slope(m.x); a4[1] *= lrelu_slope(m.y); a4[2] *= lrelu_slope(m.z); a4[3] *= lrelu_slope(m.w);
        }
    } else {
#pragma unroll
        for (int s = 0; s < 4; ++s) {
            const int kc = (TAIL && kk + s >= ke) ? ke - 1 : kk + s;
            const size_t o = arow + kc * sa_k;
            float v = A[o];
            if (MASK) v *= lrelu_slope(am[o]);
            a4[s] = (TAIL && kk + s >= ke) ? 0.f : v;
        }
    }
    if (VB && !TAIL) {
        const float4 t = *reinterpret_cast<const float4*>(Bm + bcol + kk);
        b4[0] = t.x; b4[1] = t.y; b4[2] = t.z; b4[3] = t.w;
    } else {
#pragma unroll
        for (int s = 0; s < 4; ++s) {
            const int kc = (TAIL && kk + s >= ke) ? ke - 1 : kk + s;
            const float v = Bm[kc * sb_k + bcol];
            b4[s] = (TAIL && kk + s >= ke) ? 0.f : v;
        }
    }
}
template <int U, bool VA, bool VB, bool MASK>
__device__ __forceinline__ f32x4 gemm_wave_slice(const float* __restrict__ A, const float* __restrict__ am, const float* __restrict__ Bm,
                                                 size_t arow, size_t sa_k, size_t bcol, size_t sb_k, int kb, int ke, int q) {
    f32x4 acc = {0.f, 0.f, 0.f, 0.f};
    int k = kb;
    for (; k + 16 * U <= ke; k += 16 * U) {
        float a[U][4], b[U][4];
#pragma unroll
        for (int u = 0; u < U; ++u) gemm_step_load<VA, VB, MASK, false>(A, am, Bm, arow, sa_k, bcol, sb_k, k + 16 * u + 4 * q, ke, a[u], b[u]);
#pragma unroll
        for (int u = 0; u < U; ++u)
#pragma unroll
            for (int s = 0; s < 4; ++s) acc = __builtin_amdgcn_mfma_f32_16x16x4f32(a[u][s], b[u][s], acc, 0, 0, 0);
    }
    for (; k + 16 <= ke; k += 16) {
        float a[4], b[4];
        gemm_step_load<VA, VB, MASK, false>(A, am, Bm, arow, sa_k, bcol, sb_k, k + 4 * q, ke, a, b);
#pragma unroll
        for (int s = 0; s < 4; ++s) acc = __builtin_amdgcn_mfma_f32_16x16x4f32(a[s], b[s], acc, 0, 0, 0);
    }
    if (k < ke) {
        float a[4], b[4];
        gemm_step_load<VA, VB, MASK, true>(A, am, Bm, arow, sa_k, bcol, sb_k, k + 4 * q, ke, a, b);
#pragma unroll
        for (int s = 0; s < 4; ++s) acc = __builtin_amdgcn_mfma_f32_16x16x4f32(a[s], b[s], acc, 0, 0, 0);
    }
    return acc;
}
template <int U>
__global__ __launch_bounds__(256) void gemm_f32_kernel(const float* __restrict__ A, const float* __restrict__ Bm, float* __restrict__ Cm,
                                                       int M, int N, int K, int ta, int tb, float alpha, GemmFuse fu) {
    __shared__ float red[4][16][17];
    const int lane = threadIdx.x & 63, wave = threadIdx.x >> 6, q = lane >> 4, l15 = lane & 15;
    const int i0 = blockIdx.y * 16, j0 = blockIdx.x * 16;
    const int ic = i0 + l15 < M ? i0 + l15 : M - 1, jc = j0 + l15 < N ? j0 + l15 : N - 1;
    const int kz = ((K + (int)gridDim.z - 1) / (int)gridDim.z + 15) / 16 * 16;
    const int kz0 = blockIdx.z * kz, kz1 = (kz0 + kz < K) ? kz0 + kz : K;
    const int kper = (((kz1 > kz0 ? kz1 - kz0 : 0) + 3) / 4 + 15) / 16 * 16;
    const int kb = kz0 + wave * kper, ke = (kb + kper < kz1) ? kb + kper : kz1;
    Cm += (size_t)blockIdx.z * M * N;
    const size_t sa_i = ta ? 1 : (size_t)K, sa_k = ta ? (size_t)M : 1;
    const size_t sb_k = tb ? 1 : (size_t)N, sb_j = tb ? (size_t)K : 1;
    const size_t arow = ic * sa_i, bcol = jc * sb_j;
    const bool va = !ta && (K % 4 == 0), vb = tb && (K % 4 == 0);
    f32x4 acc;
#define GEMM_SLICE(VA, VB, MK) acc = gemm_wave_slice<U, VA, VB, MK>(A, fu.amask, Bm, arow, sa_k, bcol, sb_k, kb, ke, q)
    if (fu.amask) {
        if (va) { if (vb) GEMM_SLICE(true, true, true); else GEMM_SLICE(true, false, true); }
        else    { if (vb) GEMM_SLICE(false, true, true); else GEMM_SLICE(false, false, true); }
    } else {
        if (va) { if (vb) GEMM_SLICE(true, true, false); else GEMM_SLICE(true, false, false); }
        else    { if (vb) GEMM_SLICE(false, true, false); else GEMM_SLICE(false, false, false); }
    }
#undef GEMM_SLICE
#pragma unroll
    for (int r = 0; r < 4; ++r) red[wave][q * 4 + r][l15] = acc[r];
    __syncthreads();
    const int r = threadIdx.x >> 4, c = threadIdx.x & 15;
    if (threadIdx.x < 256 && i0 + r < M && j0 + c < N) {
        const float s = ((red[0][r][c] + red[1][r][c]) + red[2][r][c]) + red[3][r][c];
        float v = alpha * s;
        if (fu.bias) v += fu.bscale * fu.bias[j0 + c];
        if (fu.act == SGX_ACT_LRELU) v = lrelu(v);
        Cm[(size_t)(i0 + r) * N + j0 + c] = v;
    }
    if (fu.colsum && blockIdx.x == 0 && blockIdx.z == 0 && threadIdx.x < 16 && i0 + (int)threadIdx.x < M) {
        const int row = i0 + threadIdx.x;
        float t = 0.f;
        int k = 0;
        for (; k + 8 <= K; k += 8) {
            float v[8], m[8];
#pragma unroll
            for (int u = 0; u < 8; ++u) {
                const size_t o = row * sa_i + (k + u) * sa_k;
                v[u] = A[o];
                m[u] = fu.amask ? fu.amask[o] : 1.f;
            }
#pragma unroll
            for (int u = 0; u < 8; ++u) t += fu.amask ? v[u] * lrelu_slope(m[u]) : v[u];
        }
        for (; k < K; ++k) {
            const size_t o = row * sa_i + k * sa_k;
            t += fu.amask ? A[o] * lrelu_slope(fu.amask[o]) : A[o];
        }
        fu.colsum[row] = fu.cscale * t;
    }
}
__global__ __launch_bounds__(256) void gemm_outer_kernel(const float* __restrict__ A, const float* __restrict__ Bm, float* __restrict__ Cm,
                                                         int M, int N, int K, size_t sa_i, size_t sa_k, float alpha) {
    const size_t idx = (size_t)blockIdx.x * 256 + threadIdx.x, n4 = (size_t)N / 4;
    if (idx >= (size_t)M * n4) return;
    const size_t i = idx / n4, j = (idx % n4) * 4;
    float a[4];
    float4 b[4];
#pragma unroll
    for (int k = 0; k < 4; ++k) {
        const int kc = k < K ? k : 0;
        a[k] = A[i * sa_i + kc * sa_k];
        b[k] = *reinterpret_cast<const float4*>(Bm + (size_t)kc * N + j);
    }
    float4 acc = {0.f, 0.f, 0.f, 0.f};
#pragma unroll
    for (int k = 0; k < 4; ++k)
        if (k < K) {
            acc.x = fmaf(a[k], b[k].x, acc.x); acc.y = fmaf(a[k], b[k].y, acc.y); acc.z = fmaf(a[k], b[k].z, acc.z); acc.w = fmaf(a[k], b[k].w, acc.w);
        }
    acc.x *= alpha; acc.y *= alpha; acc.z *= alpha; acc.w *= alpha;
    *reinterpret_cast<float4*>(Cm + i * N + j) = acc;
}
__global__ void gemm_splitk_reduce(const float* __restrict__ part, float* __restrict__ Cm, int MN, int splits, float alpha) {
    const int i = blockIdx.x * blockDim.x + threadIdx.x;
    if (i >= MN) return;
    float s = 0.f;
    for (int z = 0; z < splits; ++z) s += part[(size_t)z * MN + i];
    Cm[i] = alpha * s;
}
static int gemm_splits(int M, int N, int K) {
    const int tiles = ((M + 15) / 16) * ((N + 15) / 16);
    if (tiles >= 256 || K < 1024) return 1;
    int s = K / 256, cap = (512 + tiles - 1) / tiles;
    if (s > cap) s = cap;
    return s < 1 ? 1 : s;
}
extern "C" size_t sgx_gemm_ws_bytes(int M, int N, int K) {
    const int s = gemm_splits(M, N, K);
    return s > 1 ? (size_t)s * M * N * sizeof(float) : 0;
}
static int gemm_launch(const float* A, const float* Bm, float* C, int M, int N, int K, int ta, int tb, float alpha, GemmFuse fu, void* ws,
                       size_t ws_bytes, hipStream_t st) {
    SGX_REQUIRE(M > 0 && N > 0 && K > 0, SGX_EINVAL, "gemm: bad shape %d %d %d", M, N, K);
    int splits = gemm_splits(M, N, K);
    if (splits > 1 && (!ws || ws_bytes < (size_t)splits * M * N * sizeof(float) || fu.bias || fu.act || fu.colsum)) splits = 1;
    SGX_NOTE(2.0 * M * N * K, 4.0 * ((double)M * K + (double)K * N + (double)M * N), "gemm %dx%dx%d t%d%d%s", M, N, K, ta, tb,
             fu.amask || fu.bias || fu.colsum ? " fused" : "");
    const bool fused = fu.amask || fu.bias || fu.act || fu.colsum;
    if (K <= 4 && !tb && N % 4 == 0 && !fused && ((uintptr_t)Bm | (uintptr_t)C) % 16 == 0) {
        const size_t n = (size_t)M * (N / 4);
        hipLaunchKernelGGL(gemm_outer_kernel, dim3((unsigned)((n + 255) / 256)), dim3(256), 0, st, A, Bm, C, M, N, K, ta ? (size_t)1 : (size_t)K,
                           ta ? (size_t)M : (size_t)1, alpha);
        SGX_LAUNCH_CHECK("gemm_outer");
        return 0;
    }
    const int ksplit = (K + splits - 1) / splits;
    auto kern = ksplit >= 512 ? gemm_f32_kernel<8> : gemm_f32_kernel<1>;
    if (splits == 1) {
        hipLaunchKernelGGL(kern, dim3((N + 15) / 16, (M + 15) / 16, 1), dim3(256), 0, st, A, Bm, C, M, N, K, ta, tb, alpha, fu);
        SGX_LAUNCH_CHECK("gemm_f32");
        return 0;
    }
    hipLaunchKernelGGL(kern, dim3((N + 15) / 16, (M + 15) / 16, splits), dim3(256), 0, st, A, Bm, (float*)ws, M, N, K, ta, tb, 1.0f, fu);
    SGX_LAUNCH_CHECK("gemm_f32");
    hipLaunchKernelGGL(gemm_splitk_reduce, dim3((M * N + 255) / 256), dim3(256), 0, st, (const float*)ws, C, M * N, splits, alpha);
    SGX_LAUNCH_CHECK("gemm_splitk_reduce");
    return 0;
}
extern "C" int sgx_gemm_f32(const float* A, const float* Bm, float* C, int M, int N, int K, int ta, int tb, float alpha, void* ws,
                            size_t ws_bytes, void* stream) {
    return gemm_launch(A, Bm, C, M, N, K, ta, tb, alpha, GemmFuse{nullptr, nullptr, 0.f, SGX_ACT_NONE, nullptr, 0.f}, ws, ws_bytes,
                       (hipStream_t)stream);
}
extern "C" int sgx_linear_fwd(const float* x, const float* w, const float* bias, float* y, int B, int N, int K, float w_mul, float b_mul,
                              int act, void* stream) {
    return gemm_launch(x, w, y, B, N, K, 0, 1, w_mul, GemmFuse{nullptr, bias, b_mul, act, nullptr, 0.f}, nullptr, 0, (hipStream_t)stream);
}
extern "C" int sgx_linear_bwd_data(const float* gy, const float* y_act, const float* w, float* gx, int B, int N, int K, float w_mul,
                                   void* stream) {
    return gemm_launch(gy, w, gx, B, K, N, 0, 0, w_mul, GemmFuse{y_act, nullptr, 0.f, SGX_ACT_NONE, nullptr, 0.f}, nullptr, 0,
                       (hipStream_t)stream);
}
extern "C" int sgx_linear_bwd_param(const float* gy, const float* y_act, const float* x, float* dw, float* db, int B, int N, int K,
                                    float w_mul, float b_mul, void* stream) {
    return gemm_launch(gy, x, dw, N, K, B, 1, 0, w_mul, GemmFuse{y_act, nullptr, 0.f, SGX_ACT_NONE, db, b_mul}, nullptr, 0,
                       (hipStream_t)stream);
}

#define STYLE_MAXB 32
__device__ __forceinline__ int style_group(const long long* __restrict__ tab, int G, unsigned tile) {
    if (G <= 64) {
        const int l = threadIdx.x & 63;
        const bool le = l < G && (unsigned)tab[(l < G ? l : 0) * SGX_STYLE_ROW + 4] <= tile;
        return __builtin_amdgcn_readfirstlane(__popcll(__ballot(le)) - 1);
    }
    int g = 0;
    while (g + 1 < G && (unsigned)tab[(g + 1) * SGX_STYLE_ROW + 4] <= tile) ++g;
    return g;
}
template <int MB>
__global__ __launch_bounds__(256) void style_fwd_kernel(const float* __restrict__ lm, const long long* __restrict__ tab, float* __restrict__ y,
                                                        int G, int B, int D) {
    extern __shared__ float xs[];
    const int g = style_group(tab, G, blockIdx.x);
    const long long* r = tab + (size_t)g * SGX_STYLE_ROW;
    const float* W = reinterpret_cast<const float*>(r[0]);
    const float* bias = reinterpret_cast<const float*>(r[1]);
    const int N = (int)r[2], layer = (int)r[7];
    const float w_mul = __uint_as_float((unsigned)r[5]), b_mul = __uint_as_float((unsigned)r[6]);
    const float* x = lm + (size_t)layer * B * D;
    const int col = threadIdx.x >> 4, kl = threadIdx.x & 15;
    const int n = ((int)blockIdx.x - (int)r[4]) * 16 + col;
    constexpr int STYLE_U = 8;
    const float* wrow = W + (size_t)(n < N ? n : N - 1) * D;
    float4 w[STYLE_U];
#pragma unroll
    for (int u = 0; u < STYLE_U; ++u) { const int k = kl * 4 + 64 * u; w[u] = *reinterpret_cast<const float4*>(wrow + (k < D ? k : D - 4)); }
    for (int i = threadIdx.x; i < B * D / 4; i += 256) reinterpret_cast<float4*>(xs)[i] = reinterpret_cast<const float4*>(x)[i];
    __syncthreads();
    float acc[MB];
#pragma unroll
    for (int b = 0; b < MB; ++b) acc[b] = 0.f;
    for (int k0 = kl * 4; k0 < D; k0 += 64 * STYLE_U) {
        if (k0 != kl * 4) {
#pragma unroll
            for (int u = 0; u < STYLE_U; ++u) { const int k = k0 + 64 * u; w[u] = *reinterpret_cast<const float4*>(wrow + (k < D ? k : D - 4)); }
        }
#pragma unroll
        for (int u = 0; u < STYLE_U; ++u) {
            const int k = k0 + 64 * u;
            if (k < D) {
#pragma unroll
                for (int b = 0; b < MB; ++b)
                    if (b < B) {
                        const float4 v = *reinterpret_cast<const float4*>(xs + b * D + k);
                        acc[b] += (w[u].x * v.x + w[u].y * v.y) + (w[u].z * v.z + w[u].w * v.w);
                    }
            }
        }
    }
#pragma unroll
    for (int b = 0; b < MB; ++b)
        if (b < B) {
#pragma unroll
            for (int o = 8; o > 0; o >>= 1) acc[b] += __shfl_xor(acc[b], o, 64);
        }
    if (n < N && kl == 0) {
        const float bb = bias ? b_mul * bias[n] : 0.f;
        float* yo = y + (size_t)r[3] + n;
#pragma unroll
        for (int b = 0; b < MB; ++b)
            if (b < B) yo[(size_t)b * N] = w_mul * acc[b] + bb;
    }
}
template <int MB>
// ... 67 lines not shown
        const int b = i / 64, kl = i % 64, k = blockIdx.x * 64 + kl;
        if (k < D) {
            const float sum = (part[(0 * B + b) * 64 + kl] + part[(1 * B + b) * 64 + kl]) + (part[(2 * B + b) * 64 + kl] + part[(3 * B + b) * 64 + kl]);
            glm[((size_t)layer * B + b) * D + k] = w_mul * sum;
        }
    }
}
template <int MB>
__global__ __launch_bounds__(256) void style_bwd_param_kernel(const float* __restrict__ gy, const float* __restrict__ lm,
                                                              const long long* __restrict__ tab, float* __restrict__ dw,
                                                              float* __restrict__ db, int G, int B, int D) {
    __shared__ float gs[MB][16];
    const int g = style_group(tab, G, blockIdx.x);
    const long long* r = tab + (size_t)g * SGX_STYLE_ROW;
    const int N = (int)r[2], layer = (int)r[7];
    const float w_mul = __uint_as_float((unsigned)r[5]), b_mul = __uint_as_float((unsigned)r[6]);
    const int n0 = ((int)blockIdx.x - (int)r[4]) * 16;
    const size_t noff = (size_t)r[3] / B;
    const float* gyg = gy + (size_t)r[3];
    for (int i = threadIdx.x; i < B * 16; i += 256) {
        const int b = i / 16, j = i % 16;
        gs[b][j] = (n0 + j < N) ? gyg[(size_t)b * N + n0 + j] : 0.f;
    }
    __syncthreads();
    const float* x = lm + (size_t)layer * B * D;
    for (int k = threadIdx.x; k < D; k += 256) {
        float xv[MB];
#pragma unroll
        for (int b = 0; b < MB; ++b) xv[b] = b < B ? x[(size_t)b * D + k] : 0.f;
#pragma unroll
        for (int j = 0; j < 16; ++j)
            if (n0 + j < N) {
                float s = 0.f;
#pragma unroll
                for (int b = 0; b < MB; ++b)
                    if (b < B) s += gs[b][j] * xv[b];
                dw[(noff + n0 + j) * D + k] = w_mul * s;
            }
    }
    if (db && threadIdx.x < 16 && n0 + (int)threadIdx.x < N) {
        float s = 0.f;
        for (int b = 0; b < B; ++b) s += gs[b][threadIdx.x];
        db[noff + n0 + threadIdx.x] = b_mul * s;
    }
}
static int style_check(int G, int B, int D) {
    SGX_REQUIRE(G > 0 && B > 0 && B <= STYLE_MAXB && D > 0 && D % 64 == 0, SGX_EUNSUPPORTED, "style affines: G=%d B=%d D=%d", G, B, D);
    return 0;
}
extern "C" int sgx_style_fwd(const float* lm, const void* table, float* y, int G, int B, int D, int total_tiles, void* stream) {
    int rc = style_check(G, B, D); if (rc) return rc;
    SGX_NOTE(0.0, 0.0, "style_fwd G%d B%d", G, B);
    if (B <= 4) hipLaunchKernelGGL(style_fwd_kernel<4>, dim3(total_tiles), dim3(256), (size_t)B * D * sizeof(float), (hipStream_t)stream, lm, (const long long*)table, y, G, B, D);
    else if (B <= 8) hipLaunchKernelGGL(style_fwd_kernel<8>, dim3(total_tiles), dim3(256), (size_t)B * D * sizeof(float), (hipStream_t)stream, lm, (const long long*)table, y, G, B, D);
    else if (B <= 16) hipLaunchKernelGGL(style_fwd_kernel<16>, dim3(total_tiles), dim3(256), (size_t)B * D * sizeof(float), (hipStream_t)stream, lm, (const long long*)table, y, G, B, D);
    else hipLaunchKernelGGL(style_fwd_kernel<32>, dim3(total_tiles), dim3(256), (size_t)B * D * sizeof(float), (hipStream_t)stream, lm, (const long long*)table, y, G, B, D);
    SGX_LAUNCH_CHECK("style_fwd");
    return 0;
}
extern "C" int sgx_style_bwd_data(const float* gy, const void* table, float* glm, int G, int B, int D, int max_n, void* stream) {
    int rc = style_check(G, B, D); if (rc) return rc;
    const int mb = B <= 4 ? 4 : (B <= 8 ? 8 : (B <= 16 ? 16 : 32));
    const size_t a = (size_t)mb * max_n, b = (size_t)4 * B * 64;
    SGX_NOTE(0.0, 0.0, "style_bwd_data G%d B%d", G, B);
    if (B <= 4) hipLaunchKernelGGL(style_bwd_data_kernel<4>, dim3(D / 64, G), dim3(256), (a > b ? a : b) * sizeof(float), (hipStream_t)stream, gy, (const long long*)table, glm, G, B, D);
    else if (B <= 8) hipLaunchKernelGGL(style_bwd_data_kernel<8>, dim3(D / 64, G), dim3(256), (a > b ? a : b) * sizeof(float), (hipStream_t)stream, gy, (const long long*)table, glm, G, B, D);
    else if (B <= 16) hipLaunchKernelGGL(style_bwd_data_kernel<16>, dim3(D / 64, G), dim3(256), (a > b ? a : b) * sizeof(float), (hipStream_t)stream, gy, (const long long*)table, glm, G, B, D);
    else hipLaunchKernelGGL(style_bwd_data_kernel<32>, dim3(D / 64, G), dim3(256), (a > b ? a : b) * sizeof(float), (hipStream_t)stream, gy, (const long long*)table, glm, G, B, D);
    SGX_LAUNCH_CHECK("style_bwd_data");
    return 0;
}
extern "C" int sgx_style_bwd_param(const float* gy, const float* lm, const void* table, float* dw, float* db, int G, int B, int D,
                                   int total_tiles, void* stream) {
    int rc = style_check(G, B, D); if (rc) return rc;
    SGX_NOTE(0.0, 0.0, "style_bwd_param G%d B%d", G, B);
    if (B <= 4) hipLaunchKernelGGL(style_bwd_param_kernel<4>, dim3(total_tiles), dim3(256), 0, (hipStream_t)stream, gy, lm, (const long long*)table, dw, db, G, B, D);
    else if (B <= 8) hipLaunchKernelGGL(style_bwd_param_kernel<8>, dim3(total_tiles), dim3(256), 0, (hipStream_t)stream, gy, lm, (const long long*)table, dw, db, G, B, D);
    else if (B <= 16) hipLaunchKernelGGL(style_bwd_param_kernel<16>, dim3(total_tiles), dim3(256), 0, (hipStream_t)stream, gy, lm, (const long long*)table, dw, db, G, B, D);
    else hipLaunchKernelGGL(style_bwd_param_kernel<32>, dim3(total_tiles), dim3(256), 0, (hipStream_t)stream, gy, lm, (const long long*)table, dw, db, G, B, D);
    SGX_LAUNCH_CHECK("style_bwd_param");
    return 0;
}

#define SUMSQ_BLOCKS 1024
__global__ __launch_bounds__(256) void sumsq_f32_stage1(const float* __restrict__ x, size_t n, double* __restrict__ partial) {
    __shared__ double sh[16];
    const size_t nvec = n / 4;
    double acc = 0.0;
    float part = 0.f; int cnt = 0;
    const size_t gs = (size_t)gridDim.x * 256;
    size_t i = (size_t)blockIdx.x * 256 + threadIdx.x;
    for (; i + 3 * gs < nvec; i += 4 * gs) {
        const float4 v0 = reinterpret_cast<const float4*>(x)[i], v1 = reinterpret_cast<const float4*>(x)[i + gs];
        const float4 v2 = reinterpret_cast<const float4*>(x)[i + 2 * gs], v3 = reinterpret_cast<const float4*>(x)[i + 3 * gs];
        part += ((v0.x * v0.x + v0.y * v0.y) + (v0.z * v0.z + v0.w * v0.w)) + ((v1.x * v1.x + v1.y * v1.y) + (v1.z * v1.z + v1.w * v1.w));
        part += ((v2.x * v2.x + v2.y * v2.y) + (v2.z * v2.z + v2.w * v2.w)) + ((v3.x * v3.x + v3.y * v3.y) + (v3.z * v3.z + v3.w * v3.w));
        if (++cnt == 4) { acc += (double)part; part = 0.f; cnt = 0; }
    }
    for (; i < nvec; i += gs) {
        const float4 v = reinterpret_cast<const float4*>(x)[i];
        part += (v.x * v.x + v.y * v.y) + (v.z * v.z + v.w * v.w);
    }
    if (blockIdx.x == 0 && threadIdx.x == 0)
        for (size_t i = nvec * 4; i < n; ++i) part += x[i] * x[i];
    acc += (double)part;
    const double s = block_sum_d(acc, sh);
    if (threadIdx.x == 0) partial[blockIdx.x] = s;
}
__global__ __launch_bounds__(256) void sumsq_f32_stage2(const double* __restrict__ partial, int nblk, float* __restrict__ out) {
    __shared__ double sh[16];
    double acc = 0.0;
    for (int i = threadIdx.x; i < nblk; i += 256) acc += partial[i];
    const double s = block_sum_d(acc, sh);
    if (threadIdx.x == 0) out[0] = (float)s;
}
extern "C" size_t sgx_sumsq_ws_bytes(void) { return SUMSQ_BLOCKS * sizeof(double); }
extern "C" int sgx_sumsq_f32(const float* x, size_t n, void* ws, size_t ws_bytes, float* out, void* stream) {
    SGX_REQUIRE(ws_bytes >= SUMSQ_BLOCKS * sizeof(double), SGX_EWORKSPACE, "sumsq: workspace");
    int nblk = (int)((n / 4 + 255) / 256);
    if (nblk > SUMSQ_BLOCKS) nblk = SUMSQ_BLOCKS;
    if (nblk < 1) nblk = 1;
    hipLaunchKernelGGL(sumsq_f32_stage1, dim3(nblk), dim3(256), 0, (hipStream_t)stream, x, n, (double*)ws);
    SGX_LAUNCH_CHECK("sumsq_stage1");
    hipLaunchKernelGGL(sumsq_f32_stage2, dim3(1), dim3(256), 0, (hipStream_t)stream, (const double*)ws, nblk, out);
    SGX_LAUNCH_CHECK("sumsq_stage2");
    return 0;
}
__device__ __forceinline__ float softplus_f(float x) { return x > 20.f ? x : log1pf(expf(x)); }
__device__ __forceinline__ float sigmoid_f(float x) { return 1.f / (1.f + expf(-x)); }
__global__ void logistic_loss_kernel(const float* __restrict__ fake, int nf, const float* __restrict__ real, int nr, float scale, int gen,
                                     float* __restrict__ loss, float* __restrict__ gfake, float* __restrict__ greal) {
    const int l = threadIdx.x;
    float sf = 0.f, sr = 0.f;
    const float sgn = gen ? -1.f : 1.f;
    for (int i = l; i < nf; i += 64) {
        const float x = sgn * fake[i];
        sf += softplus_f(x);
        gfake[i] = sgn * scale * sigmoid_f(x) / (float)nf;
    }
    for (int i = l; i < nr; i += 64) {
        const float x = -real[i];
        sr += softplus_f(x);
        greal[i] = -scale * sigmoid_f(x) / (float)nr;
    }
    sf = wave_sum(sf); sr = wave_sum(sr);
    if (l == 0) loss[0] = scale * (sf / (float)(nf > 0 ? nf : 1) + (nr > 0 ? sr / (float)nr : 0.f));
}
extern "C" int sgx_logistic_loss(const float* fake, int n_fake, const float* real, int n_real, float scale, int generator, float* loss,
                                 float* g_fake, float* g_real, void* stream) {
    SGX_REQUIRE(fake && n_fake > 0 && loss && g_fake, SGX_EINVAL, "logistic_loss: fake logits, loss and g_fake are required");
    SGX_REQUIRE(generator ? n_real == 0 : (real && g_real && n_real > 0), SGX_EINVAL, "logistic_loss: real logits %s", generator ? "are not part of the generator loss" : "are required");
    hipLaunchKernelGGL(logistic_loss_kernel, dim3(1), dim3(64), 0, (hipStream_t)stream, fake, n_fake, real, n_real, scale, generator, loss, g_fake, g_real);
    SGX_LAUNCH_CHECK("logistic_loss");
    return 0;
}
__global__ void scale_dev_kernel(const float* __restrict__ x, const float* __restrict__ s, float alpha, float* __restrict__ out, size_t n) {
    const float k = alpha * s[0];
    const size_t nvec = n / 4;
    for (size_t i = (size_t)blockIdx.x * blockDim.x + threadIdx.x; i < nvec; i += (size_t)gridDim.x * blockDim.x) {
        float4 v = reinterpret_cast<const float4*>(x)[i];
        v.x *= k; v.y *= k; v.z *= k; v.w *= k;
        reinterpret_cast<float4*>(out)[i] = v;
    }
    if (blockIdx.x == 0 && threadIdx.x == 0)
        for (size_t i = nvec * 4; i < n; ++i) out[i] = k * x[i];
}
// ... 9 lines not shown
```

### stylegan/pytorch_amd/functional.py

```python
import contextlib
import functools
import os
import weakref

import numpy as np
import torch
from torch.autograd import Function
from torch.autograd.function import once_differentiable

from . import native as N

_DATA_GRAD_ONLY = 0


@contextlib.contextmanager
def data_grad_only():
    global _DATA_GRAD_ONLY
    _DATA_GRAD_ONLY += 1
    try:
        yield
    finally:
        _DATA_GRAD_ONLY -= 1


# ... 938 lines not shown
        ctx.save_for_backward(x, weight, None, None, x_pre, x_pre_bits, bits, alpha if dev else None, pimg, wr)
        return y

    @staticmethod
    def backward(ctx, g):
        g = _c(g)
        bits, alpha_dev, pimg, wr = ctx.saved_tensors[6:10]
        alpha, beta, ws, bs = ctx.fade
        br = ctx.br_ref()
        need_img = ctx.needs_input_grad[3]
        want_w = ctx.needs_input_grad[4] and not _DATA_GRAD_ONLY
        want_b = br is not None and ctx.needs_input_grad[5] and not _DATA_GRAD_ONLY
        gpimg = gwr = gbr = None
        if torch.is_grad_enabled() and FUSE_FADE_BWD2 and not want_w and not want_b:
            gy, gpimg = FadeRgbBwdFn.apply(g, bits, pimg, wr, ws, alpha, beta, alpha_dev, bool(need_img))
        elif torch.is_grad_enabled():
            if alpha_dev is not None:
                g_res = _bcall(ScaleDevFn, g, alpha_dev[1:2])
                gy = _bcall(LReluBwdBitsFn, g, bits, 0.2, alpha_dev[0:1])
            else:
                g_res = g if beta == 1.0 else _bcall(ScaleFn, g, beta)
                gy = _bcall(LReluBwdBitsFn, g, bits, 0.2, alpha)
            if need_img:
                gpimg = _bcall(RgbOutFn, g_res, wr, None, ws)
            if want_w:
                gwr = _bcall(RgbWgradFn, pimg, g_res, wr, ws)
            if want_b:
                gbr = _bcall(ColSumFn, g_res, bs)
        else:
            L = N.lib()
            C = g.shape[-1]
            npix = g.numel() // C
            accum = _ACCUM_PARAM_GRADS and wr.is_leaf and (br is None or br.is_leaf)
            acc = 0
            dw = db = None
            if want_w and accum and wr.grad is not None:
                dw, acc = wr.grad, acc | 1
            if want_b and accum and br.grad is not None:
                db, acc = br.grad, acc | 2
            gy = torch.empty_like(g)
            if need_img:
                gpimg = torch.empty_like(pimg)
            wsb = L.sgx_fade_rgb_bwd_ws_bytes(npix, C)
            wsp = N.workspace(wsb, g.device)
            dev = alpha_dev is not None
            side = _PARAM_GRAD_STREAM if (accum and (want_w or want_b)) else None
            cur_raw = N.stream()
            if side is not None and side.cuda_stream == cur_raw:
                side = None
            if side is None:
                if want_w and dw is None:
                    dw = torch.empty(wr.shape, dtype=torch.float32, device=g.device)
                if want_b and db is None:
                    db = torch.empty(br.shape, dtype=torch.float32, device=g.device)
            N.check(L.sgx_fade_rgb_bwd(N.ptr(g), N.ptr(bits), N.ptr(pimg), N.ptr(_c(wr.detach())), ws, bs, 0.0 if dev else alpha, 0.0 if dev else beta,
                                       alpha_dev.data_ptr() if dev else None, N.ptr(gy), None if side is not None else N.ptr(dw),
                                       None if side is not None else N.ptr(db), acc, N.ptr(gpimg), N.ptr(wsp), wsb, npix, C,
                                       N.dt(g), cur_raw), "sgx_fade_rgb_bwd")
            if side is not None:
                fresh = []

                def finish():
                    nonlocal dw, db
                    if want_w and dw is None:
                        dw = torch.empty(wr.shape, dtype=torch.float32, device=g.device); fresh.append(dw)
                    if want_b and db is None:
                        db = torch.empty(br.shape, dtype=torch.float32, device=g.device); fresh.append(db)
                    N.check(L.sgx_fade_rgb_bwd_finish(N.ptr(wsp), wsb, npix, C, ws, bs, 0.0 if dev else beta, alpha_dev.data_ptr() if dev else None,
                                                      N.ptr(dw), N.ptr(db), acc, N.stream()), "sgx_fade_rgb_bwd_finish")
                _fork_to(side, cur_raw, finish, reads=(wsp,) + ((alpha_dev,) if dev else ()), fresh=fresh)
            if accum:
                for p_, d_ in ((wr, dw), (br, db)):
                    if d_ is not None:
                        if p_.grad is None:
                            p_.grad = d_
                        if GRAD_NOTE is not None:
                            GRAD_NOTE(p_)
            else:
                gwr, gbr = dw, db
        out = ConvFn.backward(ctx, gy)
        return (out[0], out[1], out[2], gpimg, gwr, gbr) + (None,) * 9


class ColSumFn(Function):

    @staticmethod
    def forward(ctx, x, scale):
        x = _c(x)
        C = x.shape[-1]
        npix = x.numel() // C
        out = torch.empty((C,), dtype=torch.float32, device=x.device)
        L = N.lib()
        ws = N.workspace(L.sgx_colsum_ws_bytes(npix, C), x.device)
        N.check(L.sgx_colsum(N.ptr(x), N.ptr(out), float(scale), N.ptr(ws), ws.numel(), npix, C, N.dt(x), N.stream()), "sgx_colsum")
        ctx.shape, ctx.dtype, ctx.scale = x.shape, x.dtype, float(scale)
        return out

    @staticmethod
    def backward(ctx, g):
        return (g * ctx.scale).to(ctx.dtype).expand(ctx.shape), None


class BiasActFn(Function):

    @staticmethod
    def forward(ctx, x, bias, bscale, act):
        x = _c(x)
        C = x.shape[-1]
        y = torch.empty_like(x)
        N.check(N.lib().sgx_bias_act(N.ptr(x), N.ptr(None if bias is None else _c(bias.detach())), float(bscale), N.ptr(y),
                                     x.numel() // C, C, act, N.dt(x), N.stream()), "sgx_bias_act")
        ctx.act, ctx.has_bias, ctx.bscale = act, bias is not None, float(bscale)
        ctx.save_for_backward(y if act else None)
        return y

    @staticmethod
    def backward(ctx, g):
        (y,) = ctx.saved_tensors
        g = _c(g)
        if ctx.act:
            g = _bcall(LReluBwdFn, g, y, 0.0 if ctx.act == N.ACT_RELU else 0.2, 1.0)
        gb = None
        if ctx.has_bias and ctx.needs_input_grad[1] and not _DATA_GRAD_ONLY:
            gb = _bcall(ColSumFn, g, ctx.bscale)
        return g, gb, None, None


class ScaleFn(Function):
    @staticmethod
    def forward(ctx, x, s):
        x = _c(x)
        out = torch.empty_like(x)
        N.check(N.lib().sgx_axpby(N.ptr(x), None, N.ptr(out), float(s), 0.0, x.numel(), N.dt(x), N.stream()), "sgx_axpby")
        ctx.s = float(s)
        return out

    @staticmethod
    def backward(ctx, g):
        return _bcall(ScaleFn, g, ctx.s), None


class AxpbyFn(Function):

    @staticmethod
    def forward(ctx, a, b, alpha, beta, a_act=False):
        a, b = _c(a), _c(b)
        assert a.shape == b.shape and a.dtype == b.dtype
        out = torch.empty_like(a)
        N.check(N.lib().sgx_axpby(N.ptr(a), N.ptr(b), N.ptr(out), float(alpha), float(beta), a.numel(), N.dt(a), N.stream()), "sgx_axpby")
        ctx.alpha, ctx.beta, ctx.a_act = float(alpha), float(beta), bool(a_act)
        ctx.save_for_backward(a if a_act else None)
        return out

    @staticmethod
    def backward(ctx, g):
        (a,) = ctx.saved_tensors
        ga = gb = None
        if ctx.needs_input_grad[0]:
            ga = _bcall(LReluBwdFn, g, a, 0.2, ctx.alpha) if ctx.a_act else _bcall(ScaleFn, g, ctx.alpha)
        if ctx.needs_input_grad[1]:
            gb = g if ctx.beta == 1.0 else _bcall(ScaleFn, g, ctx.beta)
        return ga, gb, None, None, None


class ScaleDevFn(Function):

    @staticmethod
    def forward(ctx, x, s):
        x = _c(x)
        out = torch.empty_like(x)
        N.check(N.lib().sgx_axpby_dev(N.ptr(x), None, N.ptr(out), s.data_ptr(), None, x.numel(), N.dt(x), N.stream()), "sgx_axpby_dev")
        ctx.s = s
        return out

    @staticmethod
    def backward(ctx, g):
        return _bcall(ScaleDevFn, g, ctx.s), None


class FadeFn(Function):

    @staticmethod
    def forward(ctx, a, b, ab, a_act=False):
        a, b = _c(a), _c(b)
        assert a.shape == b.shape and a.dtype == b.dtype and ab.dtype == torch.float32 and ab.numel() == 2 and ab.is_contiguous()
        out = torch.empty_like(a)
        N.check(N.lib().sgx_axpby_dev(N.ptr(a), N.ptr(b), N.ptr(out), ab.data_ptr(), ab.data_ptr() + 4, a.numel(), N.dt(a), N.stream()),
                "sgx_axpby_dev")
        ctx.ab, ctx.a_act = ab, bool(a_act)
        ctx.save_for_backward(a if a_act else None)
        return out

    @staticmethod
    def backward(ctx, g):
        (a,) = ctx.saved_tensors
        ga = gb = None
        if ctx.needs_input_grad[0]:
            ga = _bcall(LReluBwdFn, g, a, 0.2, ctx.ab[0:1]) if ctx.a_act else _bcall(ScaleDevFn, g, ctx.ab[0:1])
        if ctx.needs_input_grad[1]:
            gb = _bcall(ScaleDevFn, g, ctx.ab[1:2])
        return ga, gb, None, None


def fade(a, b, alpha, a_act=False, b_prescaled=False):
    if isinstance(alpha, torch.Tensor):
        assert not b_prescaled
        return call(FadeFn, a, b, alpha, bool(a_act))
# ... 553 lines not shown
        dx = torch.empty_like(x)
        N.check(N.lib().sgx_mbstd_bwd(N.ptr(gy), N.ptr(x), N.ptr(dx), B, H * W, C, gy.shape[3], N.dt(x), N.stream()), "sgx_mbstd_bwd")
        ctx.save_for_backward(gy, x)
        return dx

    @staticmethod
    @once_differentiable
    def backward(ctx, ggx):
        gy, x = ctx.saved_tensors
        ggx = _c(ggx)
        B, H, W, C = x.shape
        ddy = torch.empty_like(gy)
        gx = torch.empty_like(x)
        N.check(N.lib().sgx_mbstd_bwd2(N.ptr(ggx), N.ptr(gy), N.ptr(x), N.ptr(ddy), N.ptr(gx), B, H * W, C, gy.shape[3], N.dt(x),
                                       N.stream()), "sgx_mbstd_bwd2")
        return ddy, gx


def _dense_view(x):
    if x.is_contiguous():
        return x, None
    if x.dim() == 4 and x.permute(0, 2, 3, 1).is_contiguous():
        return x.permute(0, 2, 3, 1), (0, 3, 1, 2)
    return x.contiguous(), None


class SumSqFn(Function):

    @staticmethod
    def forward(ctx, x):
        xv, back = _dense_view(x.detach())
        if xv.dtype != torch.float32:
            raise N.SgxError("SumSqFn expects fp32 (image gradients)")
        L = N.lib()
        out = torch.empty((), dtype=torch.float32, device=x.device)
        ws = N.workspace(L.sgx_sumsq_ws_bytes(), x.device)
        N.check(L.sgx_sumsq_f32(N.ptr(xv), xv.numel(), N.ptr(ws), ws.numel(), N.ptr(out), N.stream()), "sgx_sumsq_f32")
        ctx.back = back
        ctx.save_for_backward(xv)
        return out

    @staticmethod
    @once_differentiable
    def backward(ctx, g):
        (xv,) = ctx.saved_tensors
        gx = torch.empty_like(xv)
        N.check(N.lib().sgx_scale_dev_f32(N.ptr(xv), N.ptr(_c(g.float())), 2.0, N.ptr(gx), xv.numel(), N.stream()), "sgx_scale_dev_f32")
        return gx if ctx.back is None else gx.permute(*ctx.back)


class LogisticLossFn(Function):

    @staticmethod
    def forward(ctx, fake, real, scale, generator):
        f = _c(fake.detach().reshape(-1))
        r = None if real is None else _c(real.detach().reshape(-1))
        if f.dtype != torch.float32 or (r is not None and r.dtype != torch.float32):
            raise N.SgxError("LogisticLossFn: fp32 logits expected")
        loss = torch.empty((), dtype=torch.float32, device=f.device)
        gf = torch.empty_like(f)
        gr = None if r is None else torch.empty_like(r)
        N.check(N.lib().sgx_logistic_loss(N.ptr(f), f.numel(), N.ptr(r), 0 if r is None else r.numel(), float(scale), int(bool(generator)),
                                          N.ptr(loss), N.ptr(gf), N.ptr(gr), N.stream()), "sgx_logistic_loss")
        ctx.save_for_backward(gf, gr)
        ctx.shapes = (fake.shape, None if real is None else real.shape)
        return loss

    @staticmethod
    @once_differentiable
    def backward(ctx, g):
        gf, gr = ctx.saved_tensors
        g = _c(g.float())
        out = []
        for t, shape in zip((gf, gr), ctx.shapes):
            if t is None:
                out.append(None)
                continue
            o = torch.empty_like(t)
            N.check(N.lib().sgx_scale_dev_f32(N.ptr(t), N.ptr(g), 1.0, N.ptr(o), t.numel(), N.stream()), "sgx_scale_dev_f32")
            out.append(o.view(shape))
        return out[0], out[1], None, None


class MatMulFn(Function):

    @staticmethod
    def forward(ctx, A, Bm, ta, tb, alpha):
        A, Bm = _c(A), _c(Bm)
        assert A.dtype == torch.float32 and Bm.dtype == torch.float32
        M, K = (A.shape[1], A.shape[0]) if ta else (A.shape[0], A.shape[1])
        K2, Nn = (Bm.shape[1], Bm.shape[0]) if tb else (Bm.shape[0], Bm.shape[1])
        assert K == K2, (A.shape, Bm.shape, ta, tb)
        C = torch.empty((M, Nn), dtype=torch.float32, device=A.device)
        wsb = N.lib().sgx_gemm_ws_bytes(M, Nn, K)
        ws = N.workspace(wsb, A.device) if wsb else None
        N.check(N.lib().sgx_gemm_f32(N.ptr(A), N.ptr(Bm), N.ptr(C), M, Nn, K, int(ta), int(tb), float(alpha), N.ptr(ws), wsb, N.stream()), "sgx_gemm_f32")
        ctx.ta, ctx.tb, ctx.alpha = int(ta), int(tb), float(alpha)
        ctx.save_for_backward(A, Bm)
        return C

    @staticmethod
    def backward(ctx, gC):
        A, Bm = ctx.saved_tensors
        ta, tb, al = ctx.ta, ctx.tb, ctx.alpha
        gA = gB = None
        if ctx.needs_input_grad[0]:
            gA = _bcall(MatMulFn, gC, Bm, 0, 1 - tb, al) if not ta else _bcall(MatMulFn, Bm, gC, tb, 1, al)
        if ctx.needs_input_grad[1] and not _DATA_GRAD_ONLY:
            gB = _bcall(MatMulFn, A, gC, 1 - ta, 0, al) if not tb else _bcall(MatMulFn, gC, A, 1, ta, al)
        return gA, gB, None, None, None


class LinearFn(Function):

    @staticmethod
    def forward(ctx, x, weight, bias, w_mul, b_mul, act):
        x, weight = _c(x), _c(weight)
        assert x.dtype == torch.float32 and weight.dtype == torch.float32 and x.dim() == 2
        B, K = x.shape
        Nn = weight.shape[0]
        assert weight.shape[1] == K
        y = torch.empty((B, Nn), dtype=torch.float32, device=x.device)
        N.check(N.lib().sgx_linear_fwd(N.ptr(x), N.ptr(weight), None if bias is None else N.ptr(_c(bias.detach())), N.ptr(y), B, Nn, K,
                                       float(w_mul), float(b_mul), int(act), N.stream()), "sgx_linear_fwd")
        ctx.cfg = (float(w_mul), float(b_mul), int(act), bias is not None)
        ctx.save_for_backward(x, weight, y if act else None)
        return y

    @staticmethod
    @once_differentiable
    def backward(ctx, gy):
        x, weight, y = ctx.saved_tensors
        w_mul, b_mul, act, has_bias = ctx.cfg
        gy = _c(gy)
        B, K = x.shape
        Nn = weight.shape[0]
        L = N.lib()
        gx = gw = gb = None
        if ctx.needs_input_grad[0]:
            gx = torch.empty_like(x)
            N.check(L.sgx_linear_bwd_data(N.ptr(gy), N.ptr(y), N.ptr(weight), N.ptr(gx), B, Nn, K, w_mul, N.stream()), "sgx_linear_bwd_data")
        if ctx.needs_input_grad[1] or (has_bias and ctx.needs_input_grad[2]):
            gw = torch.empty_like(weight)
            gb = torch.empty((Nn,), dtype=torch.float32, device=x.device) if has_bias else None
            N.check(L.sgx_linear_bwd_param(N.ptr(gy), N.ptr(y), N.ptr(x), N.ptr(gw), N.ptr(gb), B, Nn, K, w_mul, b_mul, N.stream()),
                    "sgx_linear_bwd_param")
        return gx, gw, gb, None, None, None


def linear_fused(x, weight, bias, w_mul, b_mul, act=N.ACT_NONE):
    return call(LinearFn, x, weight, bias, float(w_mul), float(b_mul), int(act))


class SplitLayersFn(Function):

    @staticmethod
    def forward(ctx, dl):
        lm = dl.transpose(0, 1).contiguous()
        ctx.L = lm.shape[0]
        return tuple(lm.unbind(0))

    @staticmethod
    def backward(ctx, *grads):
        ref = next(g for g in grads if g is not None)
        return torch.stack([g if g is not None else torch.zeros_like(ref) for g in grads], dim=1)


class PreStyle:
    __slots__ = ("style",)

    def __init__(self, style):
        self.style = style


_STYLE_TABLES = {}


class GroupedStyleFn(Function):

    @staticmethod
    def forward(ctx, lm, meta, *params):
        G = len(meta)
        ws, bs = params[:G], params[G:]
        lm = _c(lm)
        L_, B, D = lm.shape
        key = (tuple(w.data_ptr() for w in ws), tuple(b.data_ptr() for b in bs), meta, B)
        ent = _STYLE_TABLES.get(key)
        if ent is None:
            rows, yoff, tile = [], 0, 0
            for (layer, w_mul, b_mul), w, b in zip(meta, ws, bs):
                n = w.shape[0]
                assert w.shape[1] == D and w.is_contiguous() and w.dtype == torch.float32
                rows.append([w.data_ptr(), b.data_ptr(), n, yoff, tile, int(np.float32(w_mul).view(np.uint32)),
                             int(np.float32(b_mul).view(np.uint32)), layer])
                yoff += B * n; tile += (n + 15) // 16
            table, _ = N.upload(torch.tensor(rows, dtype=torch.int64), lm.device)
            ent = _STYLE_TABLES[key] = (table, [r[2] for r in rows], [r[3] for r in rows], yoff, tile)
        table, ns, yoffs, ytotal, tiles = ent
        y = torch.empty(ytotal, dtype=torch.float32, device=lm.device)
        N.check(N.lib().sgx_style_fwd(N.ptr(lm), N.ptr(table), N.ptr(y), G, B, D, tiles, N.stream()), "sgx_style_fwd")
        ctx.ent, ctx.G, ctx.shape = ent, G, (L_, B, D)
        ctx.save_for_backward(lm)
        return tuple(y[o:o + B * n].view(B, n) for o, n in zip(yoffs, ns))

    @staticmethod
    @once_differentiable
    def backward(ctx, *gys):
        (lm,) = ctx.saved_tensors
        table, ns, yoffs, ytotal, tiles = ctx.ent
        L_, B, D = ctx.shape
        G = ctx.G
        gy = torch.cat([(g if g is not None else torch.zeros(B, n, device=lm.device)).reshape(-1) for g, n in zip(gys, ns)])
        L = N.lib()
        glm = None
        if ctx.needs_input_grad[0]:
            glm = torch.zeros_like(lm) if G < L_ else torch.empty_like(lm)
            N.check(L.sgx_style_bwd_data(N.ptr(gy), N.ptr(table), N.ptr(glm), G, B, D, max(ns), N.stream()), "sgx_style_bwd_data")
        ntot = sum(ns)
        dw = torch.empty((ntot, D), dtype=torch.float32, device=lm.device)
        db = torch.empty((ntot,), dtype=torch.float32, device=lm.device)
        N.check(L.sgx_style_bwd_param(N.ptr(gy), N.ptr(lm), N.ptr(table), N.ptr(dw), N.ptr(db), G, B, D, tiles, N.stream()),
                "sgx_style_bwd_param")
        offs = [o // B for o in yoffs]
        gws = tuple(dw[o:o + n] for o, n in zip(offs, ns))
        gbs = tuple(db[o:o + n] for o, n in zip(offs, ns))
        return (glm, None) + gws + gbs


class NoiseArena:

    def __init__(self, numel, device):
        self.buf = torch.randn(int(numel), device=device, dtype=torch.float32)
        self.off = 0

    def take(self, b, h, w):
        n = b * h * w
        if self.off + n > self.buf.numel():
            return torch.randn(b, 1, h, w, device=self.buf.device, dtype=torch.float32)
        out = self.buf[self.off:self.off + n].view(b, 1, h, w)
        self.off += n
        return out


NOISE_ARENA = None


def linear(x, weight, bias, w_mul, b_mul, act=N.ACT_NONE):
    y = call(MatMulFn, x, weight, 0, 1, w_mul)
# ... 118 lines not shown
```

### stylegan/pytorch_amd/native.py

```python
import ctypes
import os
import subprocess
import threading

import torch

_HERE = os.path.dirname(os.path.abspath(__file__))
LIB_PATH = os.environ.get("SGX_HIP_LIB") or os.path.join(_HERE, "libsgx_hip.so")
CSRC = os.path.join(_HERE, "csrc")

F32, BF16 = 0, 1
ACT_NONE, ACT_LRELU, ACT_RELU = 0, 1, 2
EPI_ACT, EPI_NORM = 1, 2
PACK_S, PACK_D, PACK_U, PACK_UF = 0, 1, 2, 3

_lib = None
_lock = threading.Lock()

c_void_p, c_int, c_float, c_size_t = ctypes.c_void_p, ctypes.c_int, ctypes.c_float, ctypes.c_size_t
P, I, F, Z = c_void_p, c_int, c_float, c_size_t

SIGNATURES = {
    "sgx_version": (I, []),
    "sgx_last_error": (ctypes.c_char_p, []),
    "sgx_clear_error": (I, []),
    "sgx_stream_wait_stream": (I, [P, P]),
    "sgx_conv3x3": (I, [P, P, P, P, I, I, I, I, I, I, P, I, P]),
    "sgx_conv_variant": (I, [I, P, P, P, P, I, I, I, I, I, I, I, I, P]),
    "sgx_conv4x4s2_down": (I, [P, P, P, P, I, I, I, I, I, I, I, P]),
    "sgx_conv4x4s2_up": (I, [P, P, P, I, I, I, I, I, I, P]),
    "sgx_wgrad_ws_bytes": (Z, [I, I, I, I, I, I]),
    "sgx_images_u8_to_nhwc": (I, [P, P, P, I, I, I, I, I, P]),
    "sgx_selftest_tr16": (I, [P, P]),
    "sgx_conv_splitk_ws_bytes": (Z, [I, I, I, I, I, I, I]),
    "sgx_conv_splitk": (I, [I, P, P, P, P, P, I, I, I, I, I, I, I, P, Z, P]),
    "sgx_conv_config": (I, [I, I, I, I, I, I, I, P]),
    "sgx_prof_start": (I, [I, I]),
    "sgx_prof_count": (I, []),
    "sgx_prof_get": (I, [I, P, I, P, P, P, P, I]),
    "sgx_pack_weight": (I, [P, P, P, I, I, I, I, F, I, P]),
    "sgx_pack_weight_multi": (I, [P, I, I, I, P]),
    "sgx_pack_weight_blocks": (I, [I, I]),
    "sgx_wgrad3x3_param": (I, [P, P, P, P, P, Z, I, I, I, I, I, I, F, I, I, I, I, P]),
    "sgx_wgrad4x4s2_param": (I, [P, P, P, P, P, Z, I, I, I, I, I, I, F, I, I, I, I, P]),
    "sgx_bias_act": (I, [P, P, F, P, Z, I, I, I, P]),
    "sgx_lrelu_bwd": (I, [P, P, P, Z, F, F, P, I, P]),
    "sgx_lrelu_bwd_bits": (I, [P, P, P, Z, F, F, P, I, P]),
    "sgx_conv4x4s2_down_fade_ok": (I, [I, I, I, I, I, I]),
    "sgx_conv4x4s2_down_fade": (I, [P, P, P, P, F, F, P, P, P, I, I, I, I, I, I, P]),
    "sgx_conv4x4s2_down_fade_rgb": (I, [P, P, P, P, P, F, P, F, F, F, F, P, P, P, I, I, I, I, I, I, P]),
    "sgx_fade_rgb_bwd_ws_bytes": (Z, [Z, I]),
    "sgx_fade_rgb_bwd": (I, [P, P, P, P, F, F, F, F, P, P, P, P, I, P, P, Z, Z, I, I, P]),
    "sgx_fade_rgb_bwd_finish": (I, [P, Z, Z, I, F, F, F, P, P, P, I, P]),
    "sgx_fade_rgb_bwd2": (I, [P, P, P, P, F, F, F, P, P, Z, I, I, P]),
    "sgx_axpby": (I, [P, P, P, F, F, Z, I, P]),
    "sgx_axpby_dev": (I, [P, P, P, P, P, Z, I, P]),
    "sgx_blur3x3": (I, [P, P, I, I, I, I, I, P]),
    "sgx_blur3x3_act": (I, [P, P, P, I, I, I, I, I, I, P]),
    "sgx_blur_kxk": (I, [P, P, P, I, I, I, I, I, I, I, I, I, P]),
    "sgx_pool2": (I, [P, P, I, I, I, I, F, I, P]),
    "sgx_up2": (I, [P, P, I, I, I, I, F, I, P]),
    "sgx_up2_add": (I, [P, P, P, I, I, I, I, F, I, P]),
    "sgx_colsum_ws_bytes": (Z, [Z, I]),
    "sgx_colsum": (I, [P, P, F, P, Z, Z, I, I, P]),
    "sgx_rgb_in": (I, [P, P, I, I, F, P, P, Z, I, I, P]),
    "sgx_rgb_in_add": (I, [P, P, I, I, F, P, P, Z, I, I, P]),
    "sgx_rgb_out": (I, [P, P, I, I, F, P, P, Z, I, I, P]),
    "sgx_downsample_fade_rgb": (I, [P, P, I, I, I, F, F, P, P]),
    "sgx_diffaug_ws_bytes": (Z, [I, I, I]),
    "sgx_diffaug": (I, [P, P, P, I, I, I, I, I, I, P, Z, P]),
    "sgx_rgb_out_fade": (I, [P, P, I, I, F, P, P, F, F, P, P, I, I, I, I, I, P]),
    "sgx_rgb_wgrad_ws_bytes": (Z, [Z, I]),
    "sgx_rgb_wgrad": (I, [P, P, P, I, I, F, P, Z, Z, I, I, P]),
    "sgx_gepi_ws_bytes": (Z, [I, I, I]),
    "sgx_gepi_fwd": (I, [P, P, P, P, P, P, P, P, P, Z, P, I, I, I, I, I, I, P]),
    "sgx_gepi_stats": (I, [P, P, P, P, P, P, P, Z, P, I, I, I, I, I, I, P]),
    "sgx_rgb_out_epi": (I, [P, P, P, P, P, P, P, P, I, I, F, P, P, F, F, P, P, I, I, I, I, I, P]),
    "sgx_rgb_wgrad_epi_ws_bytes": (Z, [I, I, I]),
    "sgx_rgb_wgrad_epi": (I, [P, P, P, P, P, P, P, P, P, P, I, I, F, F, P, Z, I, I, I, I, P]),
    "sgx_blur3x3_stats_nparts": (I, [I, I, I, I, I]),
    "sgx_conv3x3_stats_nparts": (I, [I, I, I, I, I, I]),
    "sgx_conv3x3_signbits_ok": (I, [I, I, I, I, I, I]),
    "sgx_conv3x3_signbits": (I, [P, P, P, P, P, I, I, I, I, I, I, P, I, P]),
    "sgx_blur3x3_bits": (I, [P, P, P, I, I, I, I, I, I, P]),
    "sgx_conv4x4s2_up_blur_ok": (I, [I, I, I, I, I, I]),
    "sgx_conv4x4s2_up_blur": (I, [P, P, P, P, I, I, I, I, I, I, P]),
    "sgx_conv4x4s2_up_blur_bits": (I, [P, P, P, P, I, I, I, I, I, I, P]),
    "sgx_pack_upblur": (I, [P, P, I, I, I, I, F, P]),
    "sgx_conv_upblur_ok": (I, [I, I, I, I, I, I]),
    "sgx_conv_upblur": (I, [P, P, P, P, I, I, I, I, I, I, P]),
    "sgx_rgbconv_ok": (I, [I, I, I, I, I]),
    "sgx_rgbconv_pack": (I, [P, F, P, F, P, F, P, P, I, P]),
    "sgx_rgbconv_fwd": (I, [P, P, P, P, P, I, I, I, I, I, I, I, P]),
    "sgx_rgbconv_tune": (I, [I, I, I]),
    "sgx_rgbconv_dgrad": (I, [P, P, P, I, I, I, I, I, P]),
    "sgx_rgbconv_wgrad_ws_bytes": (Z, [I, I, I, I]),
    "sgx_rgbconv_wgrad": (I, [P, P, I, P, F, P, F, P, F, P, P, P, P, I, P, Z, I, I, I, I, I, P]),
    "sgx_conv3x3_stats": (I, [P, P, P, P, P, P, P, Z, I, I, I, I, I, I, P]),
    "sgx_blur3x3_stats": (I, [P, P, P, P, P, P, Z, I, I, I, I, I, I, P]),
    "sgx_gepi_bwd": (I, [P, P, P, P, P, P, P, P, P, P, P, P, P, Z, I, I, I, I, I, P]),
    "sgx_pixelnorm_fwd": (I, [P, P, I, I, P]),
    "sgx_pixelnorm_bwd": (I, [P, P, P, I, I, P]),
    "sgx_mbstd_fwd": (I, [P, P, I, I, I, I, I, P]),
    "sgx_mbstd_bwd": (I, [P, P, P, I, I, I, I, I, P]),
    "sgx_mbstd_bwd2": (I, [P, P, P, P, P, I, I, I, I, I, P]),
    "sgx_sumsq_ws_bytes": (Z, []),
    "sgx_sumsq_f32": (I, [P, Z, P, Z, P, P]),
    "sgx_scale_dev_f32": (I, [P, P, F, P, Z, P]),
    "sgx_logistic_loss": (I, [P, I, P, I, F, I, P, P, P, P]),
    "sgx_gemm_ws_bytes": (Z, [I, I, I]),
    "sgx_gemm_f32": (I, [P, P, P, I, I, I, I, I, F, P, Z, P]),
    "sgx_linear_fwd": (I, [P, P, P, P, I, I, I, F, F, I, P]),
    "sgx_linear_bwd_data": (I, [P, P, P, P, I, I, I, F, P]),
    "sgx_linear_bwd_param": (I, [P, P, P, P, P, I, I, I, F, F, P]),
    "sgx_style_fwd": (I, [P, P, P, I, I, I, I, P]),
    "sgx_style_bwd_data": (I, [P, P, P, I, I, I, I, P]),
    "sgx_style_bwd_param": (I, [P, P, P, P, P, I, I, I, I, P]),
    "sgx_adam_multi": (I, [P, P, P, P, P, I, F, F, F, P, P, P, P]),
    "sgx_ema_multi": (I, [P, P, P, I, F, P]),
    "sgx_gradnorm_clip_coef": (I, [P, P, I, F, P, P, P]),
}


def build(verbose: bool = False) -> str:
    cmd = ["make", "-C", CSRC, "-j", str(min(8, os.cpu_count() or 1))]
    r = subprocess.run(cmd, capture_output=True, text=True)
    if r.returncode != 0:
        raise RuntimeError("building libsgx_hip.so failed:\n" + r.stdout[-4000:] + r.stderr[-4000:])
    if verbose:
        print(r.stdout[-2000:])
    return LIB_PATH


def lib():
    global _lib
    if _lib is None:
        with _lock:
            if _lib is None:
                if not os.path.exists(LIB_PATH):
                    raise RuntimeError(f"{LIB_PATH} is missing: run `python -c 'import __graft_entry__ as g; g.build()'` "
                                       "(there is no non-HIP fallback for this path)")
                l = ctypes.CDLL(LIB_PATH)
                for name, (res, args) in SIGNATURES.items():
                    fn = getattr(l, name)
                    fn.restype, fn.argtypes = res, args
                _lib = l
    return _lib


class SgxError(RuntimeError):
    pass


def check(rc: int, what: str):
    if rc != 0:
        msg = lib().sgx_last_error().decode(errors="replace")
        raise SgxError(f"{what} failed (code {rc}): {msg}")


_raw_stream = getattr(torch._C, "_cuda_getCurrentRawStream", None)
_get_device = getattr(torch._C, "_cuda_getDevice", None) or torch.cuda.current_device


def stream() -> int:
    if _raw_stream is not None:
        return _raw_stream(_get_device())
    return torch.cuda.current_stream().cuda_stream


def dt(t: torch.Tensor) -> int:
    if t.dtype == torch.float32:
        return F32
    if t.dtype == torch.bfloat16:
        return BF16
    raise TypeError(f"unsupported activation dtype {t.dtype}")


def ptr(t):
    if t is None:
        return None
    if not t.is_cuda:
        raise SgxError("libsgx_hip kernels need GPU tensors (no CPU fallback exists for this path)")
    if not t.is_contiguous():
        raise SgxError("internal: non-contiguous tensor passed to a kernel")
    return t.data_ptr()


_ARENA = []


def capturing() -> bool:
    return torch.cuda.is_available() and torch.cuda.is_current_stream_capturing()


def reserve_capture_staging(nbytes: int = 1 << 20):
    if capturing():
        return
    if not _ARENA or _ARENA[-1][0].numel() - _ARENA[-1][1] < nbytes:
        _ARENA.append([torch.empty(max(nbytes, 1 << 20), dtype=torch.uint8).pin_memory(), 0])

# ... 132 lines not shown
```

Measured before the change: 296.8 img/s.

## Fuse style mixing and NHWC-mapped GEMMs, accumulate param grads in place

After: 298.8 img/s (median of 2 runs). No clear change (+0.7%).

```diff
diff --git a/include/sgx.h b/include/sgx.h
--- a/include/sgx.h
+++ b/include/sgx.h
@@ -81,6 +81,8 @@
 size_t sgx_colsum_ws_bytes(size_t npix, int C);
 int sgx_colsum(const void* x, float* out, float scale, void* ws, size_t ws_bytes, size_t npix, int C, int dtype,
                void* stream);
+int sgx_colsum_acc(const void* x, float* out, float scale, void* ws, size_t ws_bytes, size_t npix, int C, int dtype, int accumulate,
+                   void* stream);
 
 int sgx_rgb_in(const float* img, const float* w, int sj, int sc, float wscale, const float* bias, void* y, size_t npix,
                int C, int dtype, void* stream);
@@ -150,6 +152,8 @@
 size_t sgx_gemm_ws_bytes(int M, int N, int K);
 int sgx_gemm_f32(const float* A, const float* Bm, float* C, int M, int N, int K, int ta, int tb, float alpha,
                  void* ws, size_t ws_bytes, void* stream);
+int sgx_gemm_f32_map(const void* A, const void* Bm, void* C, int M, int N, int K, int ta, int tb, float alpha, int amap, int bmap,
+                     int cmap, int hw, int ch, int accumulate, void* ws, size_t ws_bytes, void* stream);
 int sgx_linear_fwd(const float* x, const float* w, const float* bias, float* y, int B, int N, int K, float w_mul, float b_mul,
                    int act, void* stream);
 int sgx_linear_bwd_data(const float* gy, const float* y_act, const float* w, float* gx, int B, int N, int K, float w_mul,
@@ -161,6 +165,8 @@
 int sgx_style_bwd_data(const float* gy, const void* table, float* glm, int G, int B, int D, int max_n, void* stream);
 int sgx_style_bwd_param(const float* gy, const float* lm, const void* table, float* dw, float* db, int G, int B, int D,
                         int total_tiles, void* stream);
+int sgx_mix_layers_fwd(const float* w, const void* cutoff_dev, int cutoff, float* lm, int L, int B, int D, void* stream);
+int sgx_mix_layers_bwd(const float* glm, const void* cutoff_dev, int cutoff, float* gw, int L, int B, int D, void* stream);
 
 int sgx_gepi_stats(const void* x, const float* bias, const float* noise, const float* nw, float* mean, float* rstd, void* ws, size_t ws_bytes,
                    const double* pre_part, int pre_npart, int B, int HW, int C, int flags, int dtype, void* stream);
diff --git a/stylegan/pytorch_amd/Blocks.py b/stylegan/pytorch_amd/Blocks.py
--- a/stylegan/pytorch_amd/Blocks.py
+++ b/stylegan/pytorch_amd/Blocks.py
@@ -125,8 +125,10 @@
         if self.stddev_layer is not None:
             x = self.stddev_layer.forward_nhwc(x)
         x = apply_act(self.conv.forward_nhwc(x, act=fused), post)
-        b = x.shape[0]
-        flat = x.permute(0, 3, 1, 2).reshape(b, -1).float()
+        if x.dtype == torch.bfloat16:
+            flat = x
+        else:
+            flat = x.permute(0, 3, 1, 2).reshape(x.shape[0], -1).float()
         y = apply_act(self.dense0(flat, act=fused), post)
         return self.dense1(y)
 
diff --git a/stylegan/pytorch_amd/CustomLayers.py b/stylegan/pytorch_amd/CustomLayers.py
--- a/stylegan/pytorch_amd/CustomLayers.py
+++ b/stylegan/pytorch_amd/CustomLayers.py
@@ -146,6 +146,8 @@
 
     def forward(self, x, act=ACT_NONE, weight=None):
         w = self.weight if weight is None else weight
+        if x.dim() == 4 and x.dtype == torch.bfloat16:
+            return F.linear(x, w, self.bias, self.w_mul, self.b_mul, act)
         if self.first_order_only and x.dim() == 2:
             return F.linear_fused(x.float(), w, self.bias, self.w_mul, self.b_mul, act)
         return F.linear(x.float(), w, self.bias, self.w_mul, self.b_mul, act)
diff --git a/stylegan/pytorch_amd/GAN.py b/stylegan/pytorch_amd/GAN.py
--- a/stylegan/pytorch_amd/GAN.py
+++ b/stylegan/pytorch_amd/GAN.py
@@ -111,7 +111,7 @@
             if isinstance(m, EqualizedLinear):
                 m.first_order_only = True
 
-    def forward(self, x):
+    def forward(self, x, broadcast=True):
         x = x.float()
         if hasattr(self.map, 'pixel_norm'):
             x = self.map.pixel_norm(x)
@@ -121,7 +121,7 @@
                 x = dense(x, act=ACT_LRELU)
             else:
                 x = apply_act(dense(x), self._act)
-        if self.dlatent_broadcast is not None:
+        if self.dlatent_broadcast is not None and broadcast:
             x = x.unsqueeze(1).expand(-1, self.dlatent_broadcast, -1)
         return x
 
@@ -163,33 +163,45 @@
     def forward(self, dlatents_in, depth=0, alpha=0., labels_in=None):
         assert depth < self.depth, "Requested output depth cannot be produced"
         F.prepack(_conv_weights(self))
-        dl = self._styles(dlatents_in.float(), depth)
+        if isinstance(dlatents_in, F.LayerMajor):
+            lm = dlatents_in.lm
+            dl = self._styles(None, depth, lm)
+            b, dev = lm.shape[1], lm.device
+        else:
+            dl = self._styles(dlatents_in.float(), depth)
+            b, dev = dlatents_in.shape[0], dlatents_in.device
         dt = self.act_dtype
         nblocks = len(self.blocks) if self.structure == 'fixed' else depth
         prev_arena = F.NOISE_ARENA
         if any(m.noise is None for m in self._noise_layers()):
-            b = dlatents_in.shape[0]
-            F.NOISE_ARENA = F.NoiseArena(b * sum(2 * (4 << k) ** 2 for k in range(nblocks + 1)), dlatents_in.device)
+            F.NOISE_ARENA = F.NoiseArena(b * sum(2 * (4 << k) ** 2 for k in range(nblocks + 1)), dev)
         try:
             return self._forward(dl, dt, depth, alpha)
         finally:
             F.NOISE_ARENA = prev_arena
 
-    def _styles(self, dlatents, depth):
+    def _epilogues(self, depth):
         nblocks = len(self.blocks) if self.structure == 'fixed' else depth
         epis = [self.init_block.epi1, self.init_block.epi2]
         for blk in self.blocks[:nblocks]:
             epis += [blk.epi1, blk.epi2]
-        B = dlatents.shape[0]
-        ok = (getattr(self.init_block, "const_input_layer", False) and B <= 32 and dlatents.shape[2] % 64 == 0
-              and all(getattr(e, "_fusable", False) and e.style_mod is not None for e in epis))
-        if not ok:
-            return F.call(F.SplitLayersFn, dlatents)
+        return epis
+
+    def grouped_styles_ok(self, B, D, depth):
+        return (getattr(self.init_block, "const_input_layer", False) and B <= 32 and D % 64 == 0
+                and all(getattr(e, "_fusable", False) and e.style_mod is not None for e in self._epilogues(depth)))
+
+    def _styles(self, dlatents, depth, lm=None):
+        epis = self._epilogues(depth)
+        L, B, D = (lm.shape[0], lm.shape[1], lm.shape[2]) if lm is not None else (dlatents.shape[1], dlatents.shape[0], dlatents.shape[2])
+        if not self.grouped_styles_ok(B, D, depth):
+            return F.call(F.SplitLayersFn, dlatents if lm is None else lm.transpose(0, 1))
         lins = [e.style_mod.lin for e in epis]
         meta = tuple((i, float(l.w_mul), float(l.b_mul)) for i, l in enumerate(lins))
-        lm = dlatents.transpose(0, 1).contiguous()
+        if lm is None:
+            lm = dlatents.transpose(0, 1).contiguous()
         styles = F.call(F.GroupedStyleFn, lm, meta, *[l.weight for l in lins], *[l.bias for l in lins])
-        return [F.PreStyle(s) for s in styles] + [None] * (dlatents.shape[1] - len(styles))
+        return [F.PreStyle(s) for s in styles] + [None] * (L - len(styles))
 
     def _noise_layers(self):
         ls = self.__dict__.get("_sgx_noise_layers")
@@ -281,6 +293,10 @@
         mixing = self.training and self.style_mixing_prob is not None and self.style_mixing_prob > 0
         if mixing:
             latents2, mixing_cutoff = self._mixing_override or self.draw_mixing(latents_in.shape, depth, latents_in.device)
+            if (self.truncation is None and self.g_mapping.dlatent_broadcast == self.num_layers and latents_in.is_cuda
+                    and self.g_synthesis.grouped_styles_ok(latents_in.shape[0], self.g_mapping.dlatent_size, depth)):
+                w = self.g_mapping(torch.cat([latents_in, latents2.to(latents_in.dtype)], 0), broadcast=False)
+                return self.g_synthesis(F.LayerMajor(F.call(F.MixLayersFn, w, mixing_cutoff, self.num_layers)), depth, alpha)
             both = self.g_mapping(torch.cat([latents_in, latents2.to(latents_in.dtype)], 0))
             dlatents_in, dlatents2 = both[:latents_in.shape[0]], both[latents_in.shape[0]:]
         else:
diff --git a/stylegan/pytorch_amd/csrc/pointwise.hip b/stylegan/pytorch_amd/csrc/pointwise.hip
--- a/stylegan/pytorch_amd/csrc/pointwise.hip
+++ b/stylegan/pytorch_amd/csrc/pointwise.hip
@@ -1053,7 +1053,8 @@
         __syncthreads();
     }
 }
-__global__ __launch_bounds__(256) void colsum_stage2(const double* __restrict__ ws, float* __restrict__ out, int nblk, int C, float scale) {
+__global__ __launch_bounds__(256) void colsum_stage2(const double* __restrict__ ws, float* __restrict__ out, int nblk, int C, float scale,
+                                                     int accumulate) {
     __shared__ double sh[64][5];
     const int cl = threadIdx.x & 3, pl = threadIdx.x >> 2;
     const int c = blockIdx.x * 4 + cl;
@@ -1065,7 +1066,8 @@
     if (pl == 0 && c < C) {
         double t = 0.0;
         for (int k = 0; k < 64; ++k) t += sh[k][cl];
-        out[c] = (float)(t * (double)scale);
+        const float v = (float)(t * (double)scale);
+        out[c] = accumulate ? out[c] + v : v;
     }
 }
 template <typename T, int NJ>
@@ -1117,7 +1119,17 @@
 static bool colsum_vec_ok(int C, int ve) { const int cv = C / ve; return C % ve == 0 && cv >= 1 && cv <= 256 && (cv & (cv - 1)) == 0; }
 
 extern "C" size_t sgx_colsum_ws_bytes(size_t npix, int C) { (void)npix; return (size_t)COLSUM_BLOCKS * C * sizeof(double); }
+static int colsum_launch(const void* x, float* out, float scale, void* ws, size_t ws_bytes, size_t npix, int C, int dtype, int accumulate,
+                         void* stream);
 extern "C" int sgx_colsum(const void* x, float* out, float scale, void* ws, size_t ws_bytes, size_t npix, int C, int dtype, void* stream) {
+    return colsum_launch(x, out, scale, ws, ws_bytes, npix, C, dtype, 0, stream);
+}
+extern "C" int sgx_colsum_acc(const void* x, float* out, float scale, void* ws, size_t ws_bytes, size_t npix, int C, int dtype,
+                              int accumulate, void* stream) {
+    return colsum_launch(x, out, scale, ws, ws_bytes, npix, C, dtype, accumulate, stream);
+}
+static int colsum_launch(const void* x, float* out, float scale, void* ws, size_t ws_bytes, size_t npix, int C, int dtype, int accumulate,
+                         void* stream) {
     hipStream_t st = (hipStream_t)stream;
     SGX_REQUIRE(ws_bytes >= sgx_colsum_ws_bytes(npix, C), SGX_EWORKSPACE, "colsum: workspace");
     SGX_REQUIRE(C >= 1, SGX_EINVAL, "colsum: C=%d", C);
@@ -1132,7 +1144,7 @@
     else if (dtype == SGX_F32) hipLaunchKernelGGL(colsum_stage1<float>, dim3(nblk), dim3(256), 256 * sizeof(double), st, (const float*)x, (double*)ws, npix, C);
     else hipLaunchKernelGGL(colsum_stage1<bf16_t>, dim3(nblk), dim3(256), 256 * sizeof(double), st, (const bf16_t*)x, (double*)ws, npix, C);
     SGX_LAUNCH_CHECK("colsum_stage1");
-    hipLaunchKernelGGL(colsum_stage2, dim3((C + 3) / 4), dim3(256), 0, st, (const double*)ws, out, nblk, C, scale);
+    hipLaunchKernelGGL(colsum_stage2, dim3((C + 3) / 4), dim3(256), 0, st, (const double*)ws, out, nblk, C, scale, accumulate);
     SGX_LAUNCH_CHECK("colsum_stage2");
     return 0;
 }
diff --git a/stylegan/pytorch_amd/csrc/small.hip b/stylegan/pytorch_amd/csrc/small.hip
--- a/stylegan/pytorch_amd/csrc/small.hip
+++ b/stylegan/pytorch_amd/csrc/small.hip
@@ -217,11 +217,20 @@
 }
 
 struct GemmFuse { const float* amask; const float* bias; float bscale; int act; float* colsum; float cscale; };
-template <bool VA, bool VB, bool MASK, bool TAIL>
+struct GemmMap { int amap, bmap, cmap, hw, ch, accumulate; };
+__device__ __forceinline__ size_t gemm_map_col(int col, int hw, int ch) { return (size_t)(col % hw) * ch + col / hw; }
+template <bool VA, bool VB, bool MASK, bool TAIL, int MAP = 0>
 __device__ __forceinline__ void gemm_step_load(const float* __restrict__ A, const float* __restrict__ am, const float* __restrict__ Bm,
                                                size_t arow, size_t sa_k, size_t bcol, size_t sb_k, int kk, int ke, float (&a4)[4],
-                                               float (&b4)[4]) {
-    if (VA && !TAIL) {
+                                               float (&b4)[4], int hw = 0, int ch = 0) {
+    if (MAP == 1) {
+#pragma unroll
+        for (int s = 0; s < 4; ++s) {
+            const int kc = (TAIL && kk + s >= ke) ? ke - 1 : kk + s;
+            const float v = bf2f(reinterpret_cast<const bf16_t*>(A)[arow + gemm_map_col(kc, hw, ch)]);
+            a4[s] = (TAIL && kk + s >= ke) ? 0.f : v;
+        }
+    } else if (VA && !TAIL) {
         const float4 t = *reinterpret_cast<const float4*>(A + arow + kk);
         a4[0] = t.x; a4[1] = t.y; a4[2] = t.z; a4[3] = t.w;
         if (MASK) {
@@ -238,7 +247,14 @@
             a4[s] = (TAIL && kk + s >= ke) ? 0.f : v;
         }
     }
-    if (VB && !TAIL) {
+    if (MAP == 2) {
+#pragma unroll
+        for (int s = 0; s < 4; ++s) {
+            const int kc = (TAIL && kk + s >= ke) ? ke - 1 : kk + s;
+            const float v = bf2f(reinterpret_cast<const bf16_t*>(Bm)[kc * sb_k + bcol]);
+            b4[s] = (TAIL && kk + s >= ke) ? 0.f : v;
+        }
+    } else if (VB && !TAIL) {
         const float4 t = *reinterpret_cast<const float4*>(Bm + bcol + kk);
         b4[0] = t.x; b4[1] = t.y; b4[2] = t.z; b4[3] = t.w;
     } else {
@@ -250,15 +266,16 @@
         }
     }
 }
-template <int U, bool VA, bool VB, bool MASK>
+template <int U, bool VA, bool VB, bool MASK, int MAP = 0>
 __device__ __forceinline__ f32x4 gemm_wave_slice(const float* __restrict__ A, const float* __restrict__ am, const float* __restrict__ Bm,
-                                                 size_t arow, size_t sa_k, size_t bcol, size_t sb_k, int kb, int ke, int q) {
+                                                 size_t arow, size_t sa_k, size_t bcol, size_t sb_k, int kb, int ke, int q, int hw = 0,
+                                                 int ch = 0) {
     f32x4 acc = {0.f, 0.f, 0.f, 0.f};
     int k = kb;
     for (; k + 16 * U <= ke; k += 16 * U) {
         float a[U][4], b[U][4];
 #pragma unroll
-        for (int u = 0; u < U; ++u) gemm_step_load<VA, VB, MASK, false>(A, am, Bm, arow, sa_k, bcol, sb_k, k + 16 * u + 4 * q, ke, a[u], b[u]);
+        for (int u = 0; u < U; ++u) gemm_step_load<VA, VB, MASK, false, MAP>(A, am, Bm, arow, sa_k, bcol, sb_k, k + 16 * u + 4 * q, ke, a[u], b[u], hw, ch);
 #pragma unroll
         for (int u = 0; u < U; ++u)
 #pragma unroll
@@ -266,13 +283,13 @@
     }
     for (; k + 16 <= ke; k += 16) {
         float a[4], b[4];
-        gemm_step_load<VA, VB, MASK, false>(A, am, Bm, arow, sa_k, bcol, sb_k, k + 4 * q, ke, a, b);
+        gemm_step_load<VA, VB, MASK, false, MAP>(A, am, Bm, arow, sa_k, bcol, sb_k, k + 4 * q, ke, a, b, hw, ch);
 #pragma unroll
         for (int s = 0; s < 4; ++s) acc = __builtin_amdgcn_mfma_f32_16x16x4f32(a[s], b[s], acc, 0, 0, 0);
     }
     if (k < ke) {
         float a[4], b[4];
-        gemm_step_load<VA, VB, MASK, true>(A, am, Bm, arow, sa_k, bcol, sb_k, k + 4 * q, ke, a, b);
+        gemm_step_load<VA, VB, MASK, true, MAP>(A, am, Bm, arow, sa_k, bcol, sb_k, k + 4 * q, ke, a, b, hw, ch);
 #pragma unroll
         for (int s = 0; s < 4; ++s) acc = __builtin_amdgcn_mfma_f32_16x16x4f32(a[s], b[s], acc, 0, 0, 0);
     }
@@ -337,8 +354,42 @@
         fu.colsum[row] = fu.cscale * t;
     }
 }
+template <int U>
+__global__ __launch_bounds__(256) void gemm_map_kernel(const float* __restrict__ A, const float* __restrict__ Bm, float* __restrict__ Cm,
+                                                       int M, int N, int K, int ta, int tb, float alpha, GemmMap mp, int to_ws) {
+    __shared__ float red[4][16][17];
+    const int lane = threadIdx.x & 63, wave = threadIdx.x >> 6, q = lane >> 4, l15 = lane & 15;
+    const int i0 = blockIdx.y * 16, j0 = blockIdx.x * 16;
+    const int ic = i0 + l15 < M ? i0 + l15 : M - 1, jc = j0 + l15 < N ? j0 + l15 : N - 1;
+    const int kz = ((K + (int)gridDim.z - 1) / (int)gridDim.z + 15) / 16 * 16;
+    const int kz0 = blockIdx.z * kz, kz1 = (kz0 + kz < K) ? kz0 + kz : K;
+    const int kper = (((kz1 > kz0 ? kz1 - kz0 : 0) + 3) / 4 + 15) / 16 * 16;
+    const int kb = kz0 + wave * kper, ke = (kb + kper < kz1) ? kb + kper : kz1;
+    const size_t sa_i = ta ? 1 : (size_t)K, sa_k = ta ? (size_t)M : 1;
+    const size_t sb_k = tb ? 1 : (size_t)N, sb_j = tb ? (size_t)K : 1;
+    const size_t arow = ic * sa_i, bcol = mp.bmap ? gemm_map_col(jc, mp.hw, mp.ch) : jc * sb_j;
+    const bool vb = tb && (K % 4 == 0);
+    f32x4 acc;
+    if (mp.amap)      { if (vb) acc = gemm_wave_slice<U, false, true, false, 1>(A, nullptr, Bm, arow, sa_k, bcol, sb_k, kb, ke, q, mp.hw, mp.ch);
+                        else    acc = gemm_wave_slice<U, false, false, false, 1>(A, nullptr, Bm, arow, sa_k, bcol, sb_k, kb, ke, q, mp.hw, mp.ch); }
+    else if (mp.bmap) acc = gemm_wave_slice<U, false, false, false, 2>(A, nullptr, Bm, arow, sa_k, bcol, sb_k, kb, ke, q, mp.hw, mp.ch);
+    else if (vb)      acc = gemm_wave_slice<U, false, true, false, 0>(A, nullptr, Bm, arow, sa_k, bcol, sb_k, kb, ke, q);
+    else              acc = gemm_wave_slice<U, false, false, false, 0>(A, nullptr, Bm, arow, sa_k, bcol, sb_k, kb, ke, q);
+#pragma unroll
+    for (int r = 0; r < 4; ++r) red[wave][q * 4 + r][l15] = acc[r];
+    __syncthreads();
+    const int r = threadIdx.x >> 4, c = threadIdx.x & 15;
+    if (i0 + r < M && j0 + c < N) {
+        const float s = ((red[0][r][c] + red[1][r][c]) + red[2][r][c]) + red[3][r][c];
+        const float v = alpha * s;
+        if (to_ws) Cm[(size_t)blockIdx.z * M * N + (size_t)(i0 + r) * N + j0 + c] = v;
+        else if (mp.cmap) reinterpret_cast<bf16_t*>(Cm)[(size_t)(i0 + r) * N + gemm_map_col(j0 + c, mp.hw, mp.ch)] = f2bf(v);
+        else { float* o = Cm + (size_t)(i0 + r) * N + j0 + c; *o = mp.accumulate ? *o + v : v; }
+    }
+}
+template <bool BMAP, bool CMAP, bool ACC>
 __global__ __launch_bounds__(256) void gemm_outer_kernel(const float* __restrict__ A, const float* __restrict__ Bm, float* __restrict__ Cm,
-                                                         int M, int N, int K, size_t sa_i, size_t sa_k, float alpha) {
+                                                         int M, int N, int K, size_t sa_i, size_t sa_k, float alpha, int hw, int ch) {
     const size_t idx = (size_t)blockIdx.x * 256 + threadIdx.x, n4 = (size_t)N / 4;
     if (idx >= (size_t)M * n4) return;
     const size_t i = idx / n4, j = (idx % n4) * 4;
@@ -348,7 +399,13 @@
     for (int k = 0; k < 4; ++k) {
         const int kc = k < K ? k : 0;
         a[k] = A[i * sa_i + kc * sa_k];
-        b[k] = *reinterpret_cast<const float4*>(Bm + (size_t)kc * N + j);
+        if (BMAP) {
+            const bf16_t* b16 = reinterpret_cast<const bf16_t*>(Bm) + (size_t)kc * N;
+            b[k].x = bf2f(b16[gemm_map_col((int)j, hw, ch)]); b[k].y = bf2f(b16[gemm_map_col((int)j + 1, hw, ch)]);
+            b[k].z = bf2f(b16[gemm_map_col((int)j + 2, hw, ch)]); b[k].w = bf2f(b16[gemm_map_col((int)j + 3, hw, ch)]);
+        } else {
+            b[k] = *reinterpret_cast<const float4*>(Bm + (size_t)kc * N + j);
+        }
     }
     float4 acc = {0.f, 0.f, 0.f, 0.f};
 #pragma unroll
@@ -357,7 +414,18 @@
             acc.x = fmaf(a[k], b[k].x, acc.x); acc.y = fmaf(a[k], b[k].y, acc.y); acc.z = fmaf(a[k], b[k].z, acc.z); acc.w = fmaf(a[k], b[k].w, acc.w);
         }
     acc.x *= alpha; acc.y *= alpha; acc.z *= alpha; acc.w *= alpha;
-    *reinterpret_cast<float4*>(Cm + i * N + j) = acc;
+    if (CMAP) {
+        bf16_t* c16 = reinterpret_cast<bf16_t*>(Cm) + i * N;
+        c16[gemm_map_col((int)j, hw, ch)] = f2bf(acc.x); c16[gemm_map_col((int)j + 1, hw, ch)] = f2bf(acc.y);
+        c16[gemm_map_col((int)j + 2, hw, ch)] = f2bf(acc.z); c16[gemm_map_col((int)j + 3, hw, ch)] = f2bf(acc.w);
+        return;
+    }
+    float4* o = reinterpret_cast<float4*>(Cm + i * N + j);
+    if (ACC) {
+        const float4 p = *o;
+        acc.x = p.x + acc.x; acc.y = p.y + acc.y; acc.z = p.z + acc.z; acc.w = p.w + acc.w;
+    }
+    *o = acc;
 }
 __global__ void gemm_splitk_reduce(const float* __restrict__ part, float* __restrict__ Cm, int MN, int splits, float alpha) {
     const int i = blockIdx.x * blockDim.x + threadIdx.x;
@@ -366,6 +434,16 @@
     for (int z = 0; z < splits; ++z) s += part[(size_t)z * MN + i];
     Cm[i] = alpha * s;
 }
+__global__ void gemm_splitk_reduce_map(const float* __restrict__ part, float* __restrict__ Cm, int MN, int N, int splits, float alpha,
+                                       GemmMap mp) {
+    const int i = blockIdx.x * blockDim.x + threadIdx.x;
+    if (i >= MN) return;
+    float s = 0.f;
+    for (int z = 0; z < splits; ++z) s += part[(size_t)z * MN + i];
+    const float v = alpha * s;
+    if (mp.cmap) reinterpret_cast<bf16_t*>(Cm)[(size_t)(i / N) * N + gemm_map_col(i % N, mp.hw, mp.ch)] = f2bf(v);
+    else Cm[i] = mp.accumulate ? Cm[i] + v : v;
+}
 static int gemm_splits(int M, int N, int K) {
     const int tiles = ((M + 15) / 16) * ((N + 15) / 16);
     if (tiles >= 256 || K < 1024) return 1;
@@ -378,21 +456,47 @@
     return s > 1 ? (size_t)s * M * N * sizeof(float) : 0;
 }
 static int gemm_launch(const float* A, const float* Bm, float* C, int M, int N, int K, int ta, int tb, float alpha, GemmFuse fu, void* ws,
-                       size_t ws_bytes, hipStream_t st) {
+                       size_t ws_bytes, hipStream_t st, GemmMap mp = GemmMap{0, 0, 0, 0, 0, 0}) {
     SGX_REQUIRE(M > 0 && N > 0 && K > 0, SGX_EINVAL, "gemm: bad shape %d %d %d", M, N, K);
+    const bool mapped = mp.amap || mp.bmap || mp.cmap, special = mapped || mp.accumulate;
+    if (special) {
+        SGX_REQUIRE(!(fu.amask || fu.bias || fu.act || fu.colsum), SGX_EINVAL, "gemm: map / accumulate with a fused epilogue");
+        SGX_REQUIRE(!(mp.amap && ta) && !(mp.bmap && tb) && !(mp.cmap && mp.accumulate), SGX_EINVAL, "gemm: map on a transposed operand");
+        if (mapped) {
+            SGX_REQUIRE(mp.hw > 0 && mp.ch > 0, SGX_EINVAL, "gemm: bad map %d %d", mp.hw, mp.ch);
+            SGX_REQUIRE(!mp.amap || K == mp.hw * mp.ch, SGX_EINVAL, "gemm: A map %d x %d is not K = %d", mp.hw, mp.ch, K);
+            SGX_REQUIRE(!(mp.bmap || mp.cmap) || N == mp.hw * mp.ch, SGX_EINVAL, "gemm: B / C map %d x %d is not N = %d", mp.hw, mp.ch, N);
+        }
+    }
     int splits = gemm_splits(M, N, K);
     if (splits > 1 && (!ws || ws_bytes < (size_t)splits * M * N * sizeof(float) || fu.bias || fu.act || fu.colsum)) splits = 1;
     SGX_NOTE(2.0 * M * N * K, 4.0 * ((double)M * K + (double)K * N + (double)M * N), "gemm %dx%dx%d t%d%d%s", M, N, K, ta, tb,
              fu.amask || fu.bias || fu.colsum ? " fused" : "");
     const bool fused = fu.amask || fu.bias || fu.act || fu.colsum;
-    if (K <= 4 && !tb && N % 4 == 0 && !fused && ((uintptr_t)Bm | (uintptr_t)C) % 16 == 0) {
+    if (K <= 4 && !tb && N % 4 == 0 && !fused && !mp.amap && ((uintptr_t)Bm | (uintptr_t)C) % 16 == 0) {
         const size_t n = (size_t)M * (N / 4);
-        hipLaunchKernelGGL(gemm_outer_kernel, dim3((unsigned)((n + 255) / 256)), dim3(256), 0, st, A, Bm, C, M, N, K, ta ? (size_t)1 : (size_t)K,
-                           ta ? (size_t)M : (size_t)1, alpha);
+        auto outer = mp.cmap ? (mp.bmap ? gemm_outer_kernel<true, true, false> : gemm_outer_kernel<false, true, false>)
+                   : mp.bmap ? (mp.accumulate ? gemm_outer_kernel<true, false, true> : gemm_outer_kernel<true, false, false>)
+                             : (mp.accumulate ? gemm_outer_kernel<false, false, true> : gemm_outer_kernel<false, false, false>);
+        hipLaunchKernelGGL(outer, dim3((unsigned)((n + 255) / 256)), dim3(256), 0, st, A, Bm, C, M, N, K, ta ? (size_t)1 : (size_t)K,
+                           ta ? (size_t)M : (size_t)1, alpha, mp.hw, mp.ch);
         SGX_LAUNCH_CHECK("gemm_outer");
         return 0;
     }
     const int ksplit = (K + splits - 1) / splits;
+    if (special) {
+        auto kmap = ksplit >= 512 ? gemm_map_kernel<8> : gemm_map_kernel<1>;
+        if (splits == 1) {
+            hipLaunchKernelGGL(kmap, dim3((N + 15) / 16, (M + 15) / 16, 1), dim3(256), 0, st, A, Bm, C, M, N, K, ta, tb, alpha, mp, 0);
+            SGX_LAUNCH_CHECK("gemm_map");
+            return 0;
+        }
+        hipLaunchKernelGGL(kmap, dim3((N + 15) / 16, (M + 15) / 16, splits), dim3(256), 0, st, A, Bm, (float*)ws, M, N, K, ta, tb, 1.0f, mp, 1);
+        SGX_LAUNCH_CHECK("gemm_map");
+        hipLaunchKernelGGL(gemm_splitk_reduce_map, dim3((M * N + 255) / 256), dim3(256), 0, st, (const float*)ws, C, M * N, N, splits, alpha, mp);
+        SGX_LAUNCH_CHECK("gemm_splitk_reduce_map");
+        return 0;
+    }
     auto kern = ksplit >= 512 ? gemm_f32_kernel<8> : gemm_f32_kernel<1>;
     if (splits == 1) {
         hipLaunchKernelGGL(kern, dim3((N + 15) / 16, (M + 15) / 16, 1), dim3(256), 0, st, A, Bm, C, M, N, K, ta, tb, alpha, fu);
@@ -409,6 +513,12 @@
                             size_t ws_bytes, void* stream) {
     return gemm_launch(A, Bm, C, M, N, K, ta, tb, alpha, GemmFuse{nullptr, nullptr, 0.f, SGX_ACT_NONE, nullptr, 0.f}, ws, ws_bytes,
                        (hipStream_t)stream);
+}
+extern "C" int sgx_gemm_f32_map(const void* A, const void* Bm, void* C, int M, int N, int K, int ta, int tb, float alpha, int amap, int bmap,
+                                int cmap, int hw, int ch, int accumulate, void* ws, size_t ws_bytes, void* stream) {
+    return gemm_launch((const float*)A, (const float*)Bm, (float*)C, M, N, K, ta, tb, alpha,
+                       GemmFuse{nullptr, nullptr, 0.f, SGX_ACT_NONE, nullptr, 0.f}, ws, ws_bytes, (hipStream_t)stream,
+                       GemmMap{amap != 0, bmap != 0, cmap != 0, hw, ch, accumulate != 0});
 }
 extern "C" int sgx_linear_fwd(const float* x, const float* w, const float* bias, float* y, int B, int N, int K, float w_mul, float b_mul,
                               int act, void* stream) {
@@ -642,6 +752,53 @@
     return 0;
 }
 
+__global__ __launch_bounds__(256) void mix_layers_fwd_kernel(const float* __restrict__ w, const long long* __restrict__ cut_dev, int cut,
+                                                             float* __restrict__ lm, int L, int B, int D) {
+    const size_t i = (size_t)blockIdx.x * 256 + threadIdx.x, d4 = (size_t)D / 4;
+    if (i >= (size_t)L * B * d4) return;
+    if (cut_dev) cut = (int)cut_dev[0];
+    const size_t l = i / (B * d4), rem = i % (B * d4);
+    const float* src = w + ((size_t)l < (size_t)(cut < 0 ? 0 : cut) ? 0 : (size_t)B * D);
+    reinterpret_cast<float4*>(lm)[i] = reinterpret_cast<const float4*>(src)[rem];
+}
+__global__ __launch_bounds__(256) void mix_layers_bwd_kernel(const float* __restrict__ glm, const long long* __restrict__ cut_dev, int cut,
+                                                             float* __restrict__ gw, int L, int B, int D) {
+    const size_t i = (size_t)blockIdx.x * 256 + threadIdx.x;
+    if (i >= (size_t)2 * B * D) return;
+    if (cut_dev) cut = (int)cut_dev[0];
+    const int r = (int)(i / D), d = (int)(i % D), b = r % B;
+    const bool first = r < B;
+    float acc[4] = {0.f, 0.f, 0.f, 0.f};
+    int l = 0;
+    for (; l + 4 <= L; l += 4) {
+        float v[4];
+#pragma unroll
+        for (int u = 0; u < 4; ++u) v[u] = glm[((size_t)(l + u) * B + b) * D + d];
+#pragma unroll
+        for (int u = 0; u < 4; ++u) acc[u] = acc[u] + ((((l + u < cut) == first) ? v[u] : 0.f) + 0.f);
+    }
+    for (int u = 0; l < L; ++l, ++u) acc[u] = acc[u] + ((((l < cut) == first) ? glm[((size_t)l * B + b) * D + d] : 0.f) + 0.f);
+    gw[i] = ((acc[0] + acc[1]) + acc[2]) + acc[3];
+}
+extern "C" int sgx_mix_layers_fwd(const float* w, const void* cutoff_dev, int cutoff, float* lm, int L, int B, int D, void* stream) {
+    SGX_REQUIRE(L > 0 && B > 0 && D > 0 && D % 4 == 0, SGX_EUNSUPPORTED, "mix_layers: L=%d B=%d D=%d", L, B, D);
+    SGX_NOTE(0.0, 4.0 * (2.0 * B * D + (double)L * B * D), "mix_layers_fwd L%d B%d", L, B);
+    const size_t n = (size_t)L * B * (D / 4);
+    hipLaunchKernelGGL(mix_layers_fwd_kernel, dim3((unsigned)((n + 255) / 256)), dim3(256), 0, (hipStream_t)stream, w,
+                       (const long long*)cutoff_dev, cutoff, lm, L, B, D);
+    SGX_LAUNCH_CHECK("mix_layers_fwd");
+    return 0;
+}
+extern "C" int sgx_mix_layers_bwd(const float* glm, const void* cutoff_dev, int cutoff, float* gw, int L, int B, int D, void* stream) {
+    SGX_REQUIRE(L > 0 && B > 0 && D > 0, SGX_EUNSUPPORTED, "mix_layers: L=%d B=%d D=%d", L, B, D);
+    SGX_NOTE(0.0, 4.0 * (2.0 * B * D + (double)L * B * D), "mix_layers_bwd L%d B%d", L, B);
+    const size_t n = (size_t)2 * B * D;
+    hipLaunchKernelGGL(mix_layers_bwd_kernel, dim3((unsigned)((n + 255) / 256)), dim3(256), 0, (hipStream_t)stream, glm,
+                       (const long long*)cutoff_dev, cutoff, gw, L, B, D);
+    SGX_LAUNCH_CHECK("mix_layers_bwd");
+    return 0;
+}
+
 #define SUMSQ_BLOCKS 1024
 __global__ __launch_bounds__(256) void sumsq_f32_stage1(const float* __restrict__ x, size_t n, double* __restrict__ partial) {
     __shared__ double sh[16];
diff --git a/stylegan/pytorch_amd/functional.py b/stylegan/pytorch_amd/functional.py
--- a/stylegan/pytorch_amd/functional.py
+++ b/stylegan/pytorch_amd/functional.py
@@ -1044,6 +1044,32 @@
         return (out[0], out[1], out[2], gpimg, gwr, gbr) + (None,) * 9
 
 
+def _colsum_into_grad(leaf, x, scale):
+    x = _c(x)
+    C = x.shape[-1]
+    npix = x.numel() // C
+
+    def launch():
+        L = N.lib()
+        into = leaf.grad
+        assert into is None or (into.dtype == torch.float32 and tuple(into.shape) == (C,) and into.is_contiguous())
+        out = into if into is not None else torch.empty((C,), dtype=torch.float32, device=x.device)
+        ws = N.workspace(L.sgx_colsum_ws_bytes(npix, C), x.device)
+        N.check(L.sgx_colsum_acc(N.ptr(x), N.ptr(out), float(scale), N.ptr(ws), ws.numel(), npix, C, N.dt(x), int(into is not None),
+                                 N.stream()), "sgx_colsum_acc")
+        fresh.append(out)
+    fresh = []
+    side, cur_raw = _PARAM_GRAD_STREAM, N.stream()
+    if side is None or side.cuda_stream == cur_raw:
+        launch()
+    else:
+        _fork_to(side, cur_raw, launch, reads=(x,), fresh=fresh)
+    if leaf.grad is None:
+        leaf.grad = fresh[0]
+    if GRAD_NOTE is not None:
+        GRAD_NOTE(leaf)
+
+
 class ColSumFn(Function):
 
     @staticmethod
@@ -1073,6 +1099,7 @@
         N.check(N.lib().sgx_bias_act(N.ptr(x), N.ptr(None if bias is None else _c(bias.detach())), float(bscale), N.ptr(y),
                                      x.numel() // C, C, act, N.dt(x), N.stream()), "sgx_bias_act")
         ctx.act, ctx.has_bias, ctx.bscale = act, bias is not None, float(bscale)
+        ctx.bias_ref = weakref.ref(bias) if bias is not None else (lambda: None)
         ctx.save_for_backward(y if act else None)
         return y
 
@@ -1084,7 +1111,11 @@
             g = _bcall(LReluBwdFn, g, y, 0.0 if ctx.act == N.ACT_RELU else 0.2, 1.0)
         gb = None
         if ctx.has_bias and ctx.needs_input_grad[1] and not _DATA_GRAD_ONLY:
-            gb = _bcall(ColSumFn, g, ctx.bscale)
+            bias = ctx.bias_ref()
+            if _ACCUM_PARAM_GRADS and g.dim() == 2 and bias is not None and bias.is_leaf and not torch.is_grad_enabled():
+                _colsum_into_grad(bias, g, ctx.bscale)
+            else:
+                gb = _bcall(ColSumFn, g, ctx.bscale)
         return g, gb, None, None
 
 
@@ -1804,19 +1835,65 @@
         return out[0], out[1], None, None
 
 
+def _gemm(A, Bm, ta, tb, alpha, out_map=None, into=None):
+    amap, bmap = A.dim() == 4, Bm.dim() == 4
+    geo = None
+    for t, tr in ([(A, ta)] if amap else []) + ([(Bm, tb)] if bmap else []):
+        assert t.dtype == torch.bfloat16 and not tr, "a mapped GEMM operand is bf16 and not transposed"
+        g = (t.shape[1] * t.shape[2], t.shape[3])
+        assert geo is None or geo == g
+        geo = g
+    if out_map is not None:
+        g = (out_map[1] * out_map[2], out_map[3])
+        assert geo is None or geo == g
+        geo = g
+    a2 = (A.shape[0], A[0].numel()) if amap else tuple(A.shape)
+    b2 = (Bm.shape[0], Bm[0].numel()) if bmap else tuple(Bm.shape)
+    assert (amap or A.dtype == torch.float32) and (bmap or Bm.dtype == torch.float32)
+    M, K = (a2[1], a2[0]) if ta else a2
+    K2, Nn = (b2[1], b2[0]) if tb else b2
+    assert K == K2, (A.shape, Bm.shape, ta, tb)
+    wsb = N.lib().sgx_gemm_ws_bytes(M, Nn, K)
+    ws = N.workspace(wsb, A.device) if wsb else None
+    if geo is None and into is None:
+        C = torch.empty((M, Nn), dtype=torch.float32, device=A.device)
+        N.check(N.lib().sgx_gemm_f32(N.ptr(A), N.ptr(Bm), N.ptr(C), M, Nn, K, int(ta), int(tb), float(alpha), N.ptr(ws), wsb, N.stream()), "sgx_gemm_f32")
+        return C
+    if out_map is not None:
+        assert into is None and out_map[0] == M and geo[0] * geo[1] == Nn, (out_map, M, Nn)
+        C = torch.empty(tuple(out_map), dtype=torch.bfloat16, device=A.device)
+    elif into is not None:
+        assert into.dtype == torch.float32 and tuple(into.shape) == (M, Nn) and into.is_contiguous()
+        C = into
+    else:
+        C = torch.empty((M, Nn), dtype=torch.float32, device=A.device)
+    hw, ch = geo if geo is not None else (0, 0)
+    N.check(N.lib().sgx_gemm_f32_map(N.ptr(A), N.ptr(Bm), N.ptr(C), M, Nn, K, int(ta), int(tb), float(alpha), int(amap), int(bmap),
+                                     int(out_map is not None), hw, ch, int(into is not None), N.ptr(ws), wsb, N.stream()), "sgx_gemm_f32_map")
+    return C
+
+
+def _gemm_into_grad(leaf, A, Bm, ta, tb, alpha):
+    def launch():
+        fresh.append(_gemm(A, Bm, ta, tb, alpha, into=leaf.grad))
+    fresh = []
+    side, cur_raw = _PARAM_GRAD_STREAM, N.stream()
+    if side is None or side.cuda_stream == cur_raw:
+        launch()
+    else:
+        _fork_to(side, cur_raw, launch, reads=(A, Bm), fresh=fresh)
+    if leaf.grad is None:
+        leaf.grad = fresh[0]
+    if GRAD_NOTE is not None:
+        GRAD_NOTE(leaf)
+
+
 class MatMulFn(Function):
 
     @staticmethod
-    def forward(ctx, A, Bm, ta, tb, alpha):
+    def forward(ctx, A, Bm, ta, tb, alpha, out_map=None):
         A, Bm = _c(A), _c(Bm)
-        assert A.dtype == torch.float32 and Bm.dtype == torch.float32
-        M, K = (A.shape[1], A.shape[0]) if ta else (A.shape[0], A.shape[1])
-        K2, Nn = (Bm.shape[1], Bm.shape[0]) if tb else (Bm.shape[0], Bm.shape[1])
-        assert K == K2, (A.shape, Bm.shape, ta, tb)
-        C = torch.empty((M, Nn), dtype=torch.float32, device=A.device)
-        wsb = N.lib().sgx_gemm_ws_bytes(M, Nn, K)
-        ws = N.workspace(wsb, A.device) if wsb else None
-        N.check(N.lib().sgx_gemm_f32(N.ptr(A), N.ptr(Bm), N.ptr(C), M, Nn, K, int(ta), int(tb), float(alpha), N.ptr(ws), wsb, N.stream()), "sgx_gemm_f32")
+        C = _gemm(A, Bm, ta, tb, alpha, out_map)
         ctx.ta, ctx.tb, ctx.alpha = int(ta), int(tb), float(alpha)
         ctx.save_for_backward(A, Bm)
         return C
@@ -1825,12 +1902,19 @@
     def backward(ctx, gC):
         A, Bm = ctx.saved_tensors
         ta, tb, al = ctx.ta, ctx.tb, ctx.alpha
+        gC = _c(gC)
+        a_map = tuple(A.shape) if A.dim() == 4 else None
+        b_map = tuple(Bm.shape) if Bm.dim() == 4 else None
         gA = gB = None
         if ctx.needs_input_grad[0]:
-            gA = _bcall(MatMulFn, gC, Bm, 0, 1 - tb, al) if not ta else _bcall(MatMulFn, Bm, gC, tb, 1, al)
+            gA = _bcall(MatMulFn, gC, Bm, 0, 1 - tb, al, a_map) if not ta else _bcall(MatMulFn, Bm, gC, tb, 1, al, a_map)
         if ctx.needs_input_grad[1] and not _DATA_GRAD_ONLY:
-            gB = _bcall(MatMulFn, A, gC, 1 - ta, 0, al) if not tb else _bcall(MatMulFn, gC, A, 1, ta, al)
-        return gA, gB, None, None, None
+            args = (A, gC, 1 - ta, 0, al) if not tb else (gC, A, 1, ta, al)
+            if _ACCUM_PARAM_GRADS and Bm.is_leaf and b_map is None and not torch.is_grad_enabled():
+                _gemm_into_grad(Bm, *args)
+            else:
+                gB = _bcall(MatMulFn, *args, b_map)
+        return gA, gB, None, None, None, None
 
 
 class LinearFn(Function):
@@ -1886,6 +1970,41 @@
     def backward(ctx, *grads):
         ref = next(g for g in grads if g is not None)
         return torch.stack([g if g is not None else torch.zeros_like(ref) for g in grads], dim=1)
+
+
+class LayerMajor:
+    __slots__ = ("lm",)
+
+    def __init__(self, lm):
+        self.lm = lm
+
+
+class MixLayersFn(Function):
+
+    @staticmethod
+    def forward(ctx, w, cutoff, L):
+        w = _c(w)
+        assert w.dtype == torch.float32 and w.dim() == 2 and w.shape[0] % 2 == 0
+        B, D = w.shape[0] // 2, w.shape[1]
+        dev_cut = cutoff if isinstance(cutoff, torch.Tensor) else None
+        if dev_cut is not None:
+            assert dev_cut.dtype == torch.int64 and dev_cut.numel() == 1 and dev_cut.device == w.device
+        lm = torch.empty((L, B, D), dtype=torch.float32, device=w.device)
+        N.check(N.lib().sgx_mix_layers_fwd(N.ptr(w), N.ptr(dev_cut), 0 if dev_cut is not None else int(cutoff), N.ptr(lm), L, B, D, N.stream()),
+                "sgx_mix_layers_fwd")
+        ctx.cut, ctx.dims = cutoff, (L, B, D)
+        return lm
+
+    @staticmethod
+    @once_differentiable
+    def backward(ctx, glm):
+        L, B, D = ctx.dims
+        glm = _c(glm)
+        dev_cut = ctx.cut if isinstance(ctx.cut, torch.Tensor) else None
+        gw = torch.empty((2 * B, D), dtype=torch.float32, device=glm.device)
+        N.check(N.lib().sgx_mix_layers_bwd(N.ptr(glm), N.ptr(dev_cut), 0 if dev_cut is not None else int(ctx.cut), N.ptr(gw), L, B, D, N.stream()),
+                "sgx_mix_layers_bwd")
+        return gw, None, None
 
 
 class PreStyle:
diff --git a/stylegan/pytorch_amd/native.py b/stylegan/pytorch_amd/native.py
--- a/stylegan/pytorch_amd/native.py
+++ b/stylegan/pytorch_amd/native.py
@@ -63,6 +63,7 @@
     "sgx_up2_add": (I, [P, P, P, I, I, I, I, F, I, P]),
     "sgx_colsum_ws_bytes": (Z, [Z, I]),
     "sgx_colsum": (I, [P, P, F, P, Z, Z, I, I, P]),
+    "sgx_colsum_acc": (I, [P, P, F, P, Z, Z, I, I, I, P]),
     "sgx_rgb_in": (I, [P, P, I, I, F, P, P, Z, I, I, P]),
     "sgx_rgb_in_add": (I, [P, P, I, I, F, P, P, Z, I, I, P]),
     "sgx_rgb_out": (I, [P, P, I, I, F, P, P, Z, I, I, P]),
@@ -110,12 +111,15 @@
     "sgx_logistic_loss": (I, [P, I, P, I, F, I, P, P, P, P]),
     "sgx_gemm_ws_bytes": (Z, [I, I, I]),
     "sgx_gemm_f32": (I, [P, P, P, I, I, I, I, I, F, P, Z, P]),
+    "sgx_gemm_f32_map": (I, [P, P, P, I, I, I, I, I, F, I, I, I, I, I, I, P, Z, P]),
     "sgx_linear_fwd": (I, [P, P, P, P, I, I, I, F, F, I, P]),
     "sgx_linear_bwd_data": (I, [P, P, P, P, I, I, I, F, P]),
     "sgx_linear_bwd_param": (I, [P, P, P, P, P, I, I, I, F, F, P]),
     "sgx_style_fwd": (I, [P, P, P, I, I, I, I, P]),
     "sgx_style_bwd_data": (I, [P, P, P, I, I, I, I, P]),
     "sgx_style_bwd_param": (I, [P, P, P, P, P, I, I, I, I, P]),
+    "sgx_mix_layers_fwd": (I, [P, P, I, P, I, I, I, P]),
+    "sgx_mix_layers_bwd": (I, [P, P, I, P, I, I, I, P]),
     "sgx_adam_multi": (I, [P, P, P, P, P, I, F, F, F, P, P, P, P]),
     "sgx_ema_multi": (I, [P, P, P, I, F, P]),
     "sgx_gradnorm_clip_coef": (I, [P, P, I, F, P, P, P]),
```
